# agent-charon/MinGraph-UNet

Measured on AMD Instinct MI355X. Metric: segmented Mpix/sec, full MinGraph-UNet forward (U-Net + patch-graph GAT), 512x512 batch, higher is better.
Workload: dtype f32

## Files before the change

mingraph-unet_amd/csrc/common.h:

```cpp
#pragma once
#include <hip/hip_runtime.h>
#include <stdint.h>

#include "device.h"

namespace mgu {

inline int grid_for(int64_t work, int threads, int cap) {
  int64_t b = (work + threads - 1) / threads;
  if (b < 1) b = 1;
  if (b > cap) b = cap;
  return (int)b;
}
inline bool aligned16(const void* p) { return ((uintptr_t)p & 15) == 0; }

struct Tuning {
  bool first_mfma = true;
  bool use_wino = true;
  int wino_prec = 1;
  bool convt_frag = true;
  bool wino_cp = true;
  int wino_ppb_cap = 32;
  bool wgrad_halo = true;
  bool wino_wgrad = true;
  bool convt_dgrad_x3 = true;
  bool wgrad_x3 = true;
  bool wgrad_thin = true;
  bool wino_dgrad = true;
  bool gat_fused = true;
  bool head_fused = true;
  bool wino_asm = true;
};
const Tuning& default_tuning();
hipError_t ensure_dyn_lds(const void* func, size_t bytes, bool (&done)[64]);

struct IgemmDesc {
  const Tuning* tn;
  const float* in;
  const float* w;
  const float* wu;
  const float* scale;
  const float* shift;
  float* out;
  int M;
  int H, W;
  int Cp;
  int ldin;
  int KS;
  int K;
  int Kp;
  int N;
  int ldout;
  int coff;
  int relu;
  int out_mode;
  int ct_cout;
  int Hout, Wout;
  float* pool;
  int ldpool;
  double* stat_slots;
  int split_n;
  float* out2;
  int ld2;
};

struct WinoHead {
  const float* w;
  const float* b;
  float* logits;
  float* psum;
  int ncls;
  int psum_bytes;
};
inline size_t wino_head_psum_bytes(int B, int H, int W) { return (size_t)B * (H / 16) * (W / 16) * 8 * 32 * sizeof(float); }

inline const Tuning& tun(const IgemmDesc& d) { return d.tn ? *d.tn : default_tuning(); }
enum class ConvKernel {
  None,
  WinoAsmWide, WinoAsmCp1r2, WinoAsmCp1r4,
  WinoAsmCp1r2Head,
  WinoCp2, WinoCp1, WinoCp2Stats, WinoCp1Stats,
  WinoCp1Head,
  WinoF32Wide, WinoF32Narrow,
  WinoX3Wide, WinoX3Narrow,
  HaloF32, HaloBf16Np8, HaloBf16Np4,
  TilesF32, TilesBf16,
  ConvtX3, ConvtBf16f, ConvtX3Dgrad,
};
ConvKernel pick_conv(const IgemmDesc& d, int dtype, const WinoHead* head = nullptr);
hipError_t launch_conv(const IgemmDesc& d, ConvKernel k, int dtype, hipStream_t s, const WinoHead* head = nullptr);
inline bool conv_fuses_head(ConvKernel k) { return k == ConvKernel::WinoAsmCp1r2Head || k == ConvKernel::WinoCp1Head; }
inline hipError_t launch_igemm_f32(const IgemmDesc& d, hipStream_t s) { return launch_conv(d, pick_conv(d, 0), 0, s); }
inline hipError_t launch_igemm_bf16(const IgemmDesc& d, hipStream_t s) { return launch_conv(d, pick_conv(d, 1), 1, s); }
const char* conv_kernel_name(ConvKernel k, const IgemmDesc& d);
const char* conv_dgrad_name(ConvKernel k, const IgemmDesc& d);
struct ConvCost {
  double mfma;
  int pipe;
};
ConvCost conv_cost(ConvKernel k, const IgemmDesc& d);
inline bool conv_is_wino(ConvKernel k) { return k >= ConvKernel::WinoAsmWide && k <= ConvKernel::WinoX3Narrow; }
inline bool conv_fuses_pool(ConvKernel k) {
  return conv_is_wino(k) || (k >= ConvKernel::HaloF32 && k <= ConvKernel::HaloBf16Np4);
}
inline bool conv_reads_panel(ConvKernel k) {
  return !conv_is_wino(k) && k != ConvKernel::ConvtX3 && k != ConvKernel::ConvtBf16f && k != ConvKernel::ConvtX3Dgrad;
}
bool wino_layer(const Tuning& t, int KS, int Cp);
bool wino_dgrad_layer(const Tuning& t, int KS, int Cop);
bool convt_x3_layer(const Tuning& t, int Cin, int Cout);
bool convt_x3_dgrad_layer(const Tuning& t, int Cin, int Cout);
bool convt_bf16f_layer(const Tuning& t, int Cin, int Cout);
bool wino_head_layer(const Tuning& t, int dtype, int Cin, int ncls, int patch, int B, int H, int W);
inline bool wino_wide(const IgemmDesc& d) { return d.N > 32; }
struct WinoPlan {
  int tiles_x, tiles_y, total, nblk, ppb, ngroups, per_xcd;
};
WinoPlan wino_plan(const IgemmDesc& d);
int wino_grid_blocks(const IgemmDesc& d);
hipError_t launch_convt_x3(const IgemmDesc& d, hipStream_t s);
hipError_t launch_convt_bf16f(const IgemmDesc& d, hipStream_t s);
hipError_t launch_convt_x3_dgrad(const IgemmDesc& d, hipStream_t s);
bool first_mfma_applicable(int dtype, int Cin, int Cp, int Cout, int ldout, int coff, int64_t H, int64_t W);
hipError_t launch_first_mfma(int dtype, const void* in, const float* wfm, const float* scale, const float* shift, void* out, int B, int H,
                             int W, int ldout, int coff, int relu, hipStream_t s);
hipError_t launch_first_mfma_direct(int dtype, const float* x, int64_t sn, int64_t sc, int64_t sh, int64_t sw, int cin, const float* wfm,
                                    const float* scale, const float* shift, void* out, int B, int H, int W, int ldout, int coff, int relu,
                                    hipStream_t s);
bool first_conv_applicable(int dtype, int Cin, int Cp, int Cout, int ldout, int coff);
hipError_t launch_first_conv(int dtype, const void* in, const float* wf, const float* scale, const float* shift, void* out, int B, int H, int W,
                             int Cin, int Cout, int ldout, int coff, int relu, hipStream_t s);
hipError_t launch_wino_f32(const IgemmDesc& d, ConvKernel k, hipStream_t s, const WinoHead* head = nullptr);
hipError_t launch_patch_sum_combine(const float* psum, float* out, int nodes, hipStream_t s);
hipError_t launch_wino_cp_asm(const IgemmDesc& d, ConvKernel k, hipStream_t s, const WinoHead* head = nullptr);

struct PackItem {
  const float* w;
  float* U;
  int Cout, Cin, Cp, Np, dgrad;
  unsigned blk0;
  int kind;
  int mode;
};
static_assert(sizeof(PackItem) == 48, "PackItem must have no padding");
PackItem pack_wino(const float* w, float* U, int Cout, int Cin, int Cp, int dgrad, int prec);
PackItem pack_first_w(const float* w, float* wf, int Cout, int Cin);
PackItem pack_first_mfma(const float* w, float* wfm, int Cout, int Cin);
PackItem pack_convt_x3(const float* w, float* Wx, int Cin, int Cout, int dgrad);
PackItem pack_bias_tile(const float* bias, float* shift, int C, int reps);
PackItem pack_dgrad_panel(const float* w, float* wp, int Cout, int Cin, int Cop, int KS, int Kp);
PackItem pack_conv_panel(const float* w, void* wp, int dtype, int Cout, int Cin, int Cp, int KS, int Kp);
PackItem pack_convt_panel(const float* w, void* wp, int dtype, int Cin, int Cout, int Kp);
PackItem pack_convt_bf16f(const float* w, float* Wf, int Cin, int Cout);
PackItem pack_convt_dgrad_panel(const float* w, float* wp, int Cin, int Cout, int Kp);
size_t wino_u_floats(int Cout, int Cp);
size_t convt_x3_floats(int Cin, int Cout);
size_t convt_x3_dgrad_floats(int Cin, int Cout);
size_t convt_bf16f_floats(int Cin, int Cout);
size_t first_mfma_floats();
constexpr int PACK_MAX = 64;
struct PackBatch {
  int n;
  unsigned total_blocks;
  PackItem it[PACK_MAX];
};
bool pack_batch_prepare(PackBatch& b);
hipError_t launch_pack_batch(const PackBatch* batch_dev, unsigned total_blocks, hipStream_t s);
hipError_t launch_pack_one(const PackItem& it, hipStream_t s);

struct WgradDesc {
  const Tuning* tn;
  const float* z;
  int ldz, zoff;
  const float* in;
  int ldin, inoff, Cp;
  int KS;
  int M, H, W;
  int Hs, Ws;
  int N, K, Kp;
  float* dw;
  size_t dw_capacity;
  int groups;
  int rows_per_split;
};
inline const Tuning& tun(const WgradDesc& d) { return d.tn ? *d.tn : default_tuning(); }
enum class WgradKernel {
  Thin,
  WinoX3,
  Wino,
  Halo,
  Tiles,
};
WgradKernel pick_wgrad(const WgradDesc& d);
const char* wgrad_kernel_name(WgradKernel k);
struct WgradCost {
  double mfma;
  int pipe;
};
WgradCost wgrad_cost(WgradKernel k, double alg);
hipError_t launch_wgrad_f32(WgradDesc& d, hipStream_t s);
hipError_t launch_wino_wgrad_f32(WgradDesc& d, bool x3, hipStream_t s);
hipError_t launch_wgrad_thin(WgradDesc& d, hipStream_t s);

constexpr int STAT_ROWS = 576;
constexpr int CHAN_REDUCE_ROWS = 512;
size_t chan_reduce_work_bytes(int Cmax);
hipError_t launch_bn_stats(const float* z, int ldz, int64_t M, int C, double* work, double* sums, hipStream_t s);
hipError_t launch_bn_finalize(const double* sum, const double* sumsq, int64_t M, float eps, float momentum,
                              const float* gamma, const float* beta, float* mean, float* invstd, float* scale,
                              float* shift, float* run_mean, float* run_var, int C, hipStream_t s);
hipError_t launch_bn_finalize_slots(double* slots, int nrows, double* sums, int64_t M, float eps, float momentum, const float* gamma,
                                    const float* beta, float* mean, float* invstd, float* scale, float* shift, float* run_mean,
                                    float* run_var, int C, hipStream_t s);
hipError_t launch_bn_apply_relu(const float* z, const float* scale, const float* shift, float* y, int ldy, int64_t M, int C,
                                hipStream_t s);
hipError_t launch_bn_apply_relu_pool(const float* z, const float* scale, const float* shift, float* y, int ldy, float* pooled, int B, int H,
                                     int W, int C, hipStream_t s);
hipError_t launch_bn_bwd_reduce(const float* dy, int lddy, const float* fwd_scale, const float* fwd_shift, const float* z, int ldz,
                                const float* mean, const float* invstd, int64_t M, int C, double* work, double* sums,
                                float* dbeta, float* dgamma, hipStream_t s);
hipError_t launch_bn_bwd_apply(const float* dy, int lddy, const float* fwd_scale, const float* fwd_shift, const float* z, const float* mean,
                               const float* invstd, const float* gamma, const double* sums, int64_t M, int C, float* dz,
                               double* work, float* dbias, hipStream_t s);
hipError_t launch_bn_bwd_apply_deferred(const float* dy, int lddy, const float* fsc, const float* fsh, const float* z, const float* mean,
                                        const float* invstd, const float* gamma, const double* sums, int64_t M, int C, float* dz,
                                        double* work, int* rows, hipStream_t s);
hipError_t launch_colsum(const float* z, int ldz, int64_t M, int C, double* work, float* out, hipStream_t s);
hipError_t launch_maxpool2_bwd_add(const float* y, int ldy, const float* dpool, float* dskip, int ldd, int B, int H, int W,
                                   int C, hipStream_t s);
hipError_t launch_zero_pad_region(float* buf, int ld, int coff, int C, int B, int H, int W, int h2, int w2, hipStream_t s);
hipError_t launch_ce(const float* logits, const int64_t* labels, int64_t M, int C, long long ignore_index, float grad_scale,
                     float* dlogits, int ldd, double* acc, int* err_word, float* loss_out, hipStream_t s);
hipError_t launch_unpack_conv_grad(const float* dwp, int groups, size_t panel_stride, float* g, int Cout, int Cin, int Cp, int KS,
                                   int Kp, hipStream_t s, double* fold_slots = nullptr, int fold_rows = 0, int fold_n = 0, float* fold_out = nullptr);
hipError_t launch_unpack_convt_grad(const float* dwp, int groups, size_t panel_stride, float* g, int Cin, int Cout, int Kp, hipStream_t s);
hipError_t launch_sgd(float* p, const float* g, float* buf, int64_t n, float lr, float momentum, float wd, int step, float grad_scale,
                      hipStream_t s);
hipError_t launch_adam(float* p, const float* g, float* m, float* v, int64_t n, float lr, float b1, float b2, float eps,
                       float wd, int step, float grad_scale, hipStream_t s);

hipError_t launch_pack_input(const float* x, void* out, int dtype, int B, int C, int Cp, int H, int W, int64_t sn, int64_t sc,
                             int64_t sh, int64_t sw, hipStream_t s);
hipError_t launch_maxpool2(const void* in, int ldin, void* out, int dtype, int B, int H, int W, int C, hipStream_t s);
bool patch_mean_head_fusable(int dtype, int C, int ncls);
hipError_t launch_patch_mean(const void* feat, int dtype, float* out, int B, int H, int W, int C, int patch, hipStream_t s,
                             const float* head_w = nullptr, const float* head_b = nullptr, float* logits = nullptr, int ncls = 0);
hipError_t launch_bn_fold(const float* bias, const float* gamma, const float* beta, const float* mean, const float* var,
                          float eps, float* scale, float* shift, int C, hipStream_t s);
hipError_t launch_conv1x1_head(const void* in, int dtype, int ldin, int C, const float* w, const float* bias, float* out,
                               int ldout, int ncls, int64_t npix, hipStream_t s);
hipError_t launch_argmax(const float* logits, int64_t npix, int C, int64_t* pred, hipStream_t s);

hipError_t launch_gat_wa_rows(const float* W, const float* a, float* panel, int row0, int heads, int Fh, int Fin, int Kp, hipStream_t s);
bool gat_fused_applicable(int Fin, int heads, int Fh, int64_t E);
size_t gat_fused_scratch_floats(int Fin, int heads, int Fh);
hipError_t launch_gat_prep(const float* W, const float* a, float* wa, unsigned* Wx, int heads, int Fh, int Fin, hipStream_t s);
hipError_t launch_gat_stmax(const float* x, const float* wa, int N, int Fin, int heads, const int32_t* rowptr, const int32_t* col,
                            const int32_t* gp, int G, float alpha, float* st, int32_t* node_graph, unsigned long long* gmax, int gstride,
                            unsigned gen, hipStream_t s);
hipError_t launch_gat_fused(const float* x, int Fin, const float* st, const int32_t* rowptr, const int32_t* col, const int32_t* gp, int G,
                            const unsigned long long* gmax, const unsigned* Wx, int N, int heads, int Fh, int concat, float alpha, float* out,
                            int gstride, unsigned gen, hipStream_t s);
hipError_t launch_gat_node_graph(const int32_t* gp, int G, int nodes_per_graph, int N, int32_t* node_graph, hipStream_t s);
hipError_t launch_gat_edge_max(const float* st, const int32_t* rowptr, const int32_t* col, const int32_t* node_graph, int N,
                               int heads, float alpha, unsigned long long* gmax_enc, int gstride, unsigned gen, hipStream_t s);
hipError_t launch_gat_aggregate(const float* wh, int P, const float* st, const int32_t* rowptr, const int32_t* col,
                                const int32_t* node_graph, const unsigned long long* gmax_enc, int N, int64_t E, int heads, int Fh,
                                int concat, float alpha, float* out, int gstride, unsigned gen, hipStream_t s);

}
```

mingraph-unet_amd/csrc/convt_x3.hip:

```cpp
#include <hip/hip_runtime.h>
#include <stdint.h>

#include <algorithm>
#include <type_traits>

#include "common.h"

namespace mgu {


namespace {

template <int MODE, int NI>
__global__ __launch_bounds__(256, 2) void convt2x2_x3_kernel(const float* __restrict__ in, const int ldin, const uint16_t* __restrict__ Wx,
                                                             const float* __restrict__ shift, float* __restrict__ out, const int M,
                                                             const int H, const int W, const int Cin, const int Cout, const int ldout,
                                                             const int coff, const int Hout, const int Wout, const int ntn,
                                                             const int nblocks) {
  constexpr int AP = 40, ABUF = 3 * 128 * AP;
  __shared__ __attribute__((aligned(16))) uint16_t As[2 * ABUF];
  __shared__ int rowoff[128];
  const int chunk = gridDim.x >> 3;
  const int lb = (blockIdx.x & 7) * chunk + (blockIdx.x >> 3);
  if (lb >= nblocks) return;
  const int nt = lb % ntn, mt = lb / ntn;
  const int tid = threadIdx.x, lane = tid & 63, wave = tid >> 6;
  const int wm = wave >> 1, wn = wave & 1, lr = lane & 31, lh = lane >> 5;
  const int bm0 = mt * 128;
  const int HW = H * W;
  long long pix0;
  {
    const int img = bm0 / HW, rem = bm0 - img * HW, y = rem / W;
    pix0 = ((long long)img * Hout + 2 * y) * Wout + 2 * (rem - y * W);
  }
  if (tid < 128) {
    const int m = bm0 + tid;
    int off = 0;
    if (m < M) {
      const int img = m / HW, rem = m - img * HW, y = rem / W, x = rem - y * W;
      off = (int)((((long long)img * Hout + 2 * y) * Wout + 2 * x - pix0) * ldout);
    }
    rowoff[tid] = off;
  }

  const int arow = tid >> 3, ach = (tid & 7) * 4;
  const float* aptr[4];
#pragma unroll
  for (int j = 0; j < 4; ++j) {
    const int m = min(bm0 + j * 32 + arow, M - 1);
    if (MODE == 0) {
      aptr[j] = in + (size_t)m * ldin + ach;
    } else {
      const int img = m / HW, rem = m - img * HW, y = rem / W, x = rem - y * W;
      aptr[j] = in + (((size_t)img * Hout + 2 * y) * Wout + 2 * x) * ldin + ach;
    }
  }
  const int nk = (MODE == 0 ? Cin : 4 * Cin) >> 5;
  const int spq = Cin >> 5;
  auto koff = [&](int s) -> int {
    if (MODE == 0) return s * 32;
    const int q = s / spq;
    return ((q >> 1) * Wout + (q & 1)) * ldin + (s - q * spq) * 32;
  };
  f32x4 areg[2][4];
  auto load_a = [&](int s, auto set_t) {
    constexpr int set = decltype(set_t)::value;
    const int ko = koff(s);
#pragma unroll
    for (int j = 0; j < 4; ++j) areg[set][j] = *reinterpret_cast<const f32x4*>(aptr[j] + ko);
  };
  auto store_a = [&](int buf, auto set_t) {
    constexpr int set = decltype(set_t)::value;
    uint16_t* const base = As + buf * ABUF + arow * AP + ach;
#pragma unroll
    for (int j = 0; j < 4; ++j) {
      unsigned p[3][2];
      split3_pack(areg[set][j][0], areg[set][j][1], p[0][0], p[1][0], p[2][0]);
      split3_pack(areg[set][j][2], areg[set][j][3], p[0][1], p[1][1], p[2][1]);
#pragma unroll
      for (int q = 0; q < 3; ++q) *reinterpret_cast<uint2*>(base + (q * 128 + j * 32) * AP) = uint2{p[q][0], p[q][1]};
    }
  };

  const int nt128 = NI == 2 ? nt : nt >> 1, sub0 = NI == 2 ? wn * 2 : (nt & 1) * 2 + wn;
  const u32x4* const bp = reinterpret_cast<const u32x4*>(Wx) + ((size_t)nt128 * (2 * nk) * 12 + sub0 * 3) * 64 + lane;
  u32x4 br[2][3 * NI];
  auto load_b = [&](int kk, auto buf_t) {
    constexpr int buf = decltype(buf_t)::value;
#pragma unroll
    for (int f = 0; f < 3 * NI; ++f) br[buf][f] = bp[((size_t)kk * 12 + f) * 64];
  };

  f32x16 acc[2][NI];
#pragma unroll
  for (int mi = 0; mi < 2; ++mi)
#pragma unroll
    for (int ni = 0; ni < NI; ++ni)
#pragma unroll
      for (int r = 0; r < 16; ++r) acc[mi][ni][r] = 0.f;

  const int aoff = (wm * 64 + lr) * AP + lh * 8;
  auto half_step = [&](int buf, int ss, auto bb_t) {
    constexpr int bb = decltype(bb_t)::value;
    u32x4 pa[2][3];
#pragma unroll
    for (int mi = 0; mi < 2; ++mi)
#pragma unroll
      for (int q = 0; q < 3; ++q)
        pa[mi][q] = *reinterpret_cast<const u32x4*>(As + buf * ABUF + (q * 128 + mi * 32) * AP + aoff + ss * 16);
#pragma unroll
    for (int mi = 0; mi < 2; ++mi)
#pragma unroll
      for (int ni = 0; ni < NI; ++ni) {
        f32x16 t = acc[mi][ni];
        t = mfma_bf16(pa[mi][2], br[bb][ni * 3 + 0], t);
        t = mfma_bf16(pa[mi][0], br[bb][ni * 3 + 2], t);
        t = mfma_bf16(pa[mi][1], br[bb][ni * 3 + 1], t);
        t = mfma_bf16(pa[mi][1], br[bb][ni * 3 + 0], t);
        t = mfma_bf16(pa[mi][0], br[bb][ni * 3 + 1], t);
        t = mfma_bf16(pa[mi][0], br[bb][ni * 3 + 0], t);
        acc[mi][ni] = t;
      }
  };
  using B0 = std::integral_constant<int, 0>;
  using B1 = std::integral_constant<int, 1>;
  const int nkk = 2 * nk;
  load_a(0, B0{});
  load_a(min(1, nk - 1), B1{});
  load_b(0, B0{});
  store_a(0, B0{});
  lds_barrier();
  auto second_half_and_stage = [&](int buf, auto bb_t, auto set_t) {
    half_step(buf, 1, bb_t);
    store_a(buf ^ 1, set_t);
#pragma unroll
    for (int k = 0; k < 12 * NI; ++k) {
      __builtin_amdgcn_sched_group_barrier(0x008, 1, 0);
      __builtin_amdgcn_sched_group_barrier(0x002, NI == 2 ? 4 : 8, 0);
    }
    __builtin_amdgcn_sched_group_barrier(0x200, 12, 0);
  };
  for (int s = 0; s < nk; s += 2) {
    load_a(min(s + 2, nk - 1), B0{});
    load_b(min(2 * s + 1, nkk - 1), B1{});
    __builtin_amdgcn_sched_barrier(0);
    half_step(0, 0, B0{});
    load_b(min(2 * s + 2, nkk - 1), B0{});
    __builtin_amdgcn_sched_barrier(0);
    second_half_and_stage(0, B1{}, B1{});
    __builtin_amdgcn_sched_barrier(0);
    lds_barrier();
    if (s + 1 >= nk) break;
    load_a(min(s + 3, nk - 1), B1{});
    load_b(min(2 * s + 3, nkk - 1), B1{});
    __builtin_amdgcn_sched_barrier(0);
    half_step(1, 0, B0{});
    load_b(min(2 * s + 4, nkk - 1), B0{});
    __builtin_amdgcn_sched_barrier(0);
    second_half_and_stage(1, B1{}, B0{});
    __builtin_amdgcn_sched_barrier(0);
    lds_barrier();
  }

  float* const tile_out = MODE == 0 ? out + (size_t)pix0 * ldout + coff : out + (size_t)bm0 * ldout + coff;
  const bool full_m = bm0 + 128 <= M;
  auto store_tile = [&](auto guarded_t) {
    constexpr bool GUARDED = decltype(guarded_t)::value;
#pragma unroll
    for (int ni = 0; ni < NI; ++ni) {
      const int n = nt * (64 * NI) + wn * (32 * NI) + ni * 32 + lr;
      int ncol = n;
      if (MODE == 0) {
        const int q = n / Cout;
        ncol = ((q >> 1) * Wout + (q & 1)) * ldout + (n - q * Cout);
      }
      const float sh = shift ? shift[n] : 0.f;
#pragma unroll
      for (int mi = 0; mi < 2; ++mi)
#pragma unroll
        for (int r = 0; r < 16; ++r) {
          const int rrow = wm * 64 + mi * 32 + (r & 3) + 8 * (r >> 2) + 4 * lh;
          const unsigned idx = (unsigned)((MODE == 0 ? rowoff[rrow] : rrow * ldout) + ncol);
          const float v = acc[mi][ni][r] + sh;
          if (!GUARDED) tile_out[idx] = v;
          else if (bm0 + rrow < M) tile_out[idx] = v;
        }
    }
  };
  if (full_m) store_tile(std::false_type{});
  else store_tile(std::true_type{});
}

}

hipError_t launch_convt_x3_dgrad(const IgemmDesc& d, hipStream_t s) {
  const bool wide = (d.N & 127) == 0;
  const int mtiles = (d.M + 127) / 128, ntn = d.N / (wide ? 128 : 64);
  const int nb = mtiles * ntn;
  const int chunk = (nb + 7) / 8;
  if (wide)
    hipLaunchKernelGGL((convt2x2_x3_kernel<1, 2>), dim3(chunk * 8), dim3(256), 0, s, d.in, d.ldin, reinterpret_cast<const uint16_t*>(d.wu),
                       (const float*)nullptr, d.out, d.M, d.H, d.W, d.Cp, d.N, d.ldout, d.coff, d.Hout, d.Wout, ntn, nb);
  else
    hipLaunchKernelGGL((convt2x2_x3_kernel<1, 1>), dim3(chunk * 8), dim3(256), 0, s, d.in, d.ldin, reinterpret_cast<const uint16_t*>(d.wu),
                       (const float*)nullptr, d.out, d.M, d.H, d.W, d.Cp, d.N, d.ldout, d.coff, d.Hout, d.Wout, ntn, nb);
  return hipGetLastError();
}

hipError_t launch_convt_x3(const IgemmDesc& d, hipStream_t s) {
  const int mtiles = (d.M + 127) / 128, ntn = d.N / 128;
  const int nb = mtiles * ntn;
  const int chunk = (nb + 7) / 8;
  hipLaunchKernelGGL((convt2x2_x3_kernel<0, 2>), dim3(chunk * 8), dim3(256), 0, s, d.in, d.ldin, reinterpret_cast<const uint16_t*>(d.wu), d.shift, d.out,
                     d.M, d.H, d.W, d.Cp, d.ct_cout, d.ldout, d.coff, d.Hout, d.Wout, ntn, nb);
  return hipGetLastError();
}

}
```

mingraph-unet_amd/csrc/device.h:

```cpp
#pragma once
#include <hip/hip_runtime.h>
#include <stdint.h>
#include <type_traits>

namespace mgu {

typedef float f32x16 __attribute__((ext_vector_type(16)));
typedef float f32x4 __attribute__((ext_vector_type(4)));
typedef float f32x2 __attribute__((ext_vector_type(2)));
typedef unsigned u32x4 __attribute__((ext_vector_type(4)));
typedef unsigned u32x2 __attribute__((ext_vector_type(2)));
typedef __bf16 bf16x8 __attribute__((ext_vector_type(8)));

__device__ __forceinline__ void split3_pack(const float a, const float b, unsigned& p0, unsigned& p1, unsigned& p2) {
  const unsigned ua = __float_as_uint(a), ub = __float_as_uint(b);
  p0 = __builtin_amdgcn_perm(ub, ua, 0x07060302u);
  const float ra = a - __uint_as_float(ua & 0xffff0000u), rb = b - __uint_as_float(ub & 0xffff0000u);
  const unsigned va = __float_as_uint(ra), vb = __float_as_uint(rb);
  p1 = __builtin_amdgcn_perm(vb, va, 0x07060302u);
  const float sa = ra - __uint_as_float(va & 0xffff0000u), sb = rb - __uint_as_float(vb & 0xffff0000u);
  p2 = __builtin_amdgcn_perm(__float_as_uint(sb), __float_as_uint(sa), 0x07060302u);
}
__device__ __forceinline__ float x3_add(float a, float b) {
  float d;
  asm("v_add_f32 %0, %1, %2" : "=v"(d) : "v"(a), "v"(b));
  return d;
}
__device__ __forceinline__ float x3_sub(float a, float b) {
  float d;
  asm("v_sub_f32 %0, %1, %2" : "=v"(d) : "v"(a), "v"(b));
  return d;
}
__device__ __forceinline__ float x3_fma(float a, float b, float c) {
  float d;
  asm("v_fma_f32 %0, %1, %2, %3" : "=v"(d) : "v"(a), "v"(b), "v"(c));
  return d;
}
__device__ __forceinline__ void split3_pack_s(const float a, const float b, unsigned& p0, unsigned& p1, unsigned& p2) {
  const unsigned ua = __float_as_uint(a), ub = __float_as_uint(b);
  p0 = __builtin_amdgcn_perm(ub, ua, 0x07060302u);
  const float ra = x3_sub(a, __uint_as_float(ua & 0xffff0000u)), rb = x3_sub(b, __uint_as_float(ub & 0xffff0000u));
  const unsigned va = __float_as_uint(ra), vb = __float_as_uint(rb);
  p1 = __builtin_amdgcn_perm(vb, va, 0x07060302u);
  const float sa = x3_sub(ra, __uint_as_float(va & 0xffff0000u)), sb = x3_sub(rb, __uint_as_float(vb & 0xffff0000u));
  p2 = __builtin_amdgcn_perm(__float_as_uint(sb), __float_as_uint(sa), 0x07060302u);
}

__device__ __forceinline__ f32x16 mfma_bf16(const u32x4 a, const u32x4 b, const f32x16 c) {
  return __builtin_amdgcn_mfma_f32_32x32x16_bf16(__builtin_bit_cast(bf16x8, a), __builtin_bit_cast(bf16x8, b), c, 0, 0, 0);
}

template <int I, int N, class F>
__device__ __forceinline__ void static_for(F&& f) {
  if constexpr (I < N) {
    f(std::integral_constant<int, I>{});
    static_for<I + 1, N>(f);
  }
}

__device__ __forceinline__ void lds_barrier() { asm volatile("s_waitcnt lgkmcnt(0)\n\ts_barrier" ::: "memory"); }
__device__ __forceinline__ void lds_barrier_builtin() {
  asm volatile("" ::: "memory");
  __builtin_amdgcn_s_waitcnt(0xC07F);
  __builtin_amdgcn_s_barrier();
  asm volatile("" ::: "memory");
}
__device__ __forceinline__ void lds_barrier_fenced() { __syncthreads(); }

template <typename T>
__device__ __forceinline__ T wave_sum(T v) {
#pragma unroll
  for (int off = 32; off > 0; off >>= 1) v += __shfl_xor(v, off);
  return v;
}
__device__ __forceinline__ int wave_min(int v) {
#pragma unroll
  for (int off = 32; off > 0; off >>= 1) v = min(v, __shfl_xor(v, off));
  return v;
}
__device__ __forceinline__ int wave_max(int v) {
#pragma unroll
  for (int off = 32; off > 0; off >>= 1) v = max(v, __shfl_xor(v, off));
  return v;
}
template <int K>
__device__ __forceinline__ void block_fold(double (&v)[K], double* sh ) {
#pragma unroll
  for (int k = 0; k < K; ++k)
#pragma unroll
    for (int off = 32; off > 0; off >>= 1) v[k] += __shfl_xor(v[k], off);
  const int lane = threadIdx.x & 63, wave = threadIdx.x >> 6;
  if (lane == 0)
#pragma unroll
    for (int k = 0; k < K; ++k) sh[wave * K + k] = v[k];
  __syncthreads();
  if (threadIdx.x == 0)
#pragma unroll
    for (int k = 0; k < K; ++k) v[k] = sh[k] + sh[K + k] + sh[2 * K + k] + sh[3 * K + k];
}

__device__ __forceinline__ unsigned enc_ordered(float f) {
  const unsigned u = __float_as_uint(f);
  return (u & 0x80000000u) ? ~u : (u | 0x80000000u);
}
__device__ __forceinline__ float dec_ordered(unsigned u) {
  return __uint_as_float((u & 0x80000000u) ? (u & 0x7FFFFFFFu) : ~u);
}

template <int CM>
__device__ __forceinline__ float pixel_softmax(const float* p, int C, float (&e)[CM]) {
  float l[CM];
  float m = p[0];
#pragma unroll
  for (int c = 0; c < CM; ++c)
    if (c < C) {
      l[c] = p[c];
      m = fmaxf(m, l[c]);
    }
  float sum = 0.f;
#pragma unroll
  for (int c = 0; c < CM; ++c)
    if (c < C) {
      e[c] = expf(l[c] - m);
      sum += e[c];
    }
  return sum;
}
__device__ __forceinline__ float u8_normalize(uint8_t u, int c, float m0, float m1, float m2, float s0, float s1, float s2) {
  const float v = (float)u / 255.f;
  const float mean = c == 0 ? m0 : (c == 1 ? m1 : m2), sd = c == 0 ? s0 : (c == 1 ? s1 : s2);
  return (v - mean) / sd;
}

__device__ __forceinline__ int graph_of(const int32_t* __restrict__ gp, int G, int node) {
  if (!gp || G <= 1) return 0;
  int lo = 0, hi = G;
  while (hi - lo > 1) {
    const int mid = (lo + hi) >> 1;
    if (gp[mid] <= node) lo = mid; else hi = mid;
  }
  return lo;
}

}
```

mingraph-unet_amd/csrc/igemm.hip:

```cpp
#include "common.h"
#include <algorithm>
#include <type_traits>

namespace mgu {


const Tuning& default_tuning() {
  static const Tuning t;
  return t;
}

hipError_t ensure_dyn_lds(const void* func, size_t bytes, bool (&done)[64]) {
  if (bytes <= 65536) return hipSuccess;
  int dev = 0;
  hipError_t e = hipGetDevice(&dev);
  if (e != hipSuccess) return e;
  if (dev < 0 || dev >= 64) return hipFuncSetAttribute(func, hipFuncAttributeMaxDynamicSharedMemorySize, (int)bytes);
  if (done[dev]) return hipSuccess;
  e = hipFuncSetAttribute(func, hipFuncAttributeMaxDynamicSharedMemorySize, (int)bytes);
  if (e == hipSuccess) done[dev] = true;
  return e;
}

template <typename T> struct Elem;
template <> struct Elem<float> { static constexpr int VEC = 4; };
template <> struct Elem<__bf16> { static constexpr int VEC = 8; };

template <typename T>
__device__ __forceinline__ f32x16 mma_chunk(const f32x4 a, const f32x4 b, f32x16 c) {
  if constexpr (sizeof(T) == 4) {
#pragma unroll
    for (int t = 0; t < 4; ++t) c = __builtin_amdgcn_mfma_f32_32x32x2f32(a[t], b[t], c, 0, 0, 0);
    return c;
  } else {
    return __builtin_amdgcn_mfma_f32_32x32x16_bf16(__builtin_bit_cast(bf16x8, a), __builtin_bit_cast(bf16x8, b), c, 0, 0, 0);
  }
}

template <typename T, int KS, int OUTMODE, int WAVES_M, int WAVES_N, int WMT, int WNT>
__global__ __launch_bounds__(256) void igemm_kernel(const IgemmDesc d) {
  static_assert(WAVES_M * WAVES_N == 4, "4 wavefronts per workgroup");
  constexpr int VEC = Elem<T>::VEC;
  constexpr int CK = 8 * VEC;
  constexpr int LDS_LD = CK + VEC;
  constexpr int BM = WAVES_M * WMT * 32;
  constexpr int BN = WAVES_N * WNT * 32;
  constexpr int AR = BM / 32;
  constexpr int BR = BN / 32;
  extern __shared__ __attribute__((aligned(16))) float smem_raw[];
  T* smem = reinterpret_cast<T*>(smem_raw);
  T* As = smem;
  T* Bs = smem + BM * LDS_LD;
  const T* const in_t = reinterpret_cast<const T*>(d.in);
  const T* const w_t = reinterpret_cast<const T*>(d.w);

  const int tid = threadIdx.x;
  const int lane = tid & 63;
  const int wave = tid >> 6;
  const int wm = wave / WAVES_N;
  const int wn = wave % WAVES_N;
  const int bm0 = blockIdx.x * BM;
  const int bn0 = blockIdx.y * BN;
  const int kq = tid & 7;
  const int r0 = tid >> 3;

  const T* abase[AR];
  unsigned amask[AR];
  const int HW = d.H * d.W;
#pragma unroll
  for (int i = 0; i < AR; ++i) {
    const int m = bm0 + r0 + 32 * i;
    abase[i] = in_t;
    amask[i] = 0u;
    if (m < d.M) {
      abase[i] = in_t + (size_t)m * d.ldin;
      if (KS == 2) {
        const int img = m / HW;
        const int rem = m - img * HW;
        const int oy = rem / d.W;
        const int ox = rem - oy * d.W;
        abase[i] = in_t + (((size_t)img * d.Hout + 2 * oy) * d.Wout + 2 * ox) * d.ldin;
        amask[i] = 0xFu;
      } else if (KS == 3) {
        const int rem = m % HW;
        const int oy = rem / d.W;
        const int ox = rem - oy * d.W;
        unsigned rowok = (oy > 0 ? 1u : 0u) | 2u | (oy + 1 < d.H ? 4u : 0u);
        unsigned colok = (ox > 0 ? 1u : 0u) | 2u | (ox + 1 < d.W ? 4u : 0u);
        unsigned mk = 0u;
#pragma unroll
        for (int r = 0; r < 3; ++r)
          if (rowok & (1u << r)) mk |= colok << (3 * r);
        amask[i] = mk;
      } else {
        amask[i] = 1u;
      }
    }
  }
  const T* wrow[BR];
#pragma unroll
  for (int i = 0; i < BR; ++i) wrow[i] = w_t + (size_t)(bn0 + r0 + 32 * i) * d.Kp + kq * VEC;

  f32x4 areg[AR];
  f32x4 breg[BR];
  auto load_tiles = [&](int k0) {
    const int k = k0 + kq * VEC;
    int tap = 0;
    long delta = k;
    if (KS == 3) {
      tap = k / d.Cp;
      const int c = k - tap * d.Cp;
      const int r = tap / 3;
      const int s = tap - 3 * r;
      delta = (long)((r - 1) * d.W + (s - 1)) * d.ldin + c;
    } else if (KS == 2) {
      tap = k / d.Cp;
      const int c = k - tap * d.Cp;
      delta = (long)((tap >> 1) * d.Wout + (tap & 1)) * d.ldin + c;
    }
    const bool kvalid = k < d.K;
#pragma unroll
    for (int i = 0; i < AR; ++i) {
      const bool ok = kvalid && ((amask[i] >> tap) & 1u);
      const T* src = ok ? abase[i] + delta : in_t;
      const f32x4 v = *reinterpret_cast<const f32x4*>(src);
      areg[i] = ok ? v : f32x4{0.f, 0.f, 0.f, 0.f};
    }
#pragma unroll
    for (int i = 0; i < BR; ++i) breg[i] = *reinterpret_cast<const f32x4*>(wrow[i] + k0);
  };

  f32x16 acc[WMT][WNT];
#pragma unroll
  for (int mi = 0; mi < WMT; ++mi)
#pragma unroll
    for (int ni = 0; ni < WNT; ++ni)
#pragma unroll
      for (int r = 0; r < 16; ++r) acc[mi][ni][r] = 0.f;

  const int lr = lane & 31;
  const int lh = lane >> 5;
  const T* Ap = As + (wm * WMT * 32 + lr) * LDS_LD + lh * VEC;
  const T* Bp = Bs + (wn * WNT * 32 + lr) * LDS_LD + lh * VEC;
  T* Asw = As + r0 * LDS_LD + kq * VEC;
  T* Bsw = Bs + r0 * LDS_LD + kq * VEC;

  const int nk = d.Kp / CK;
  load_tiles(0);
  for (int ks = 0; ks < nk; ++ks) {
#pragma unroll
    for (int i = 0; i < AR; ++i) *reinterpret_cast<f32x4*>(Asw + i * 32 * LDS_LD) = areg[i];
#pragma unroll
    for (int i = 0; i < BR; ++i) *reinterpret_cast<f32x4*>(Bsw + i * 32 * LDS_LD) = breg[i];
    __syncthreads();
    if (ks + 1 < nk) load_tiles((ks + 1) * CK);
#pragma unroll
    for (int kk = 0; kk < 4; ++kk) {
      if (ks * CK + kk * 2 * VEC >= d.K) break;
      f32x4 a[WMT], b[WNT];
#pragma unroll
      for (int mi = 0; mi < WMT; ++mi) a[mi] = *reinterpret_cast<const f32x4*>(Ap + mi * 32 * LDS_LD + kk * 2 * VEC);
#pragma unroll
      for (int ni = 0; ni < WNT; ++ni) b[ni] = *reinterpret_cast<const f32x4*>(Bp + ni * 32 * LDS_LD + kk * 2 * VEC);
#pragma unroll
      for (int mi = 0; mi < WMT; ++mi)
#pragma unroll
        for (int ni = 0; ni < WNT; ++ni) acc[mi][ni] = mma_chunk<T>(a[mi], b[ni], acc[mi][ni]);
    }
    __syncthreads();
  }

  int* rowoff = reinterpret_cast<int*>(smem_raw);
  long long pix0 = 0;
  if (OUTMODE == 1) {
    {
      const int img = bm0 / HW;
      const int rem = bm0 - img * HW;
      const int y = rem / d.W;
      pix0 = ((long long)img * d.Hout + 2 * y) * d.Wout + 2 * (rem - y * d.W);
    }
    for (int rrow = tid; rrow < BM; rrow += 256) {
      const int m = bm0 + rrow;
      int off = 0;
      if (m < d.M) {
        const int img = m / HW;
        const int rem = m - img * HW;
        const int y = rem / d.W;
        const int x = rem - y * d.W;
        off = (int)((((long long)img * d.Hout + 2 * y) * d.Wout + 2 * x - pix0) * d.ldout);
      }
      rowoff[rrow] = off;
    }
    __syncthreads();
  }
  const bool full_m = bm0 + BM <= d.M;
  const bool full_n = bn0 + BN <= d.N;
  T* const out_t = reinterpret_cast<T*>(d.out);
  T* const tile_out = OUTMODE == 1 ? out_t + (size_t)pix0 * d.ldout + d.coff : out_t + (size_t)bm0 * d.ldout + d.coff;
  auto store_tile = [&](auto guarded_t) {
    constexpr bool GUARDED = decltype(guarded_t)::value;
#pragma unroll
    for (int ni = 0; ni < WNT; ++ni) {
      const int n = bn0 + (wn * WNT + ni) * 32 + lr;
      const bool nvalid = n < d.N;
      const float sc = (nvalid && d.scale) ? d.scale[n] : 1.f;
      const float sh = (nvalid && d.shift) ? d.shift[n] : 0.f;
      int ncol = n;
      if (OUTMODE == 1) {
        const int q = n / d.ct_cout;
        ncol = ((q >> 1) * d.Wout + (q & 1)) * d.ldout + (n - q * d.ct_cout);
      }
      const bool split = OUTMODE == 0 && d.split_n > 0 && n >= d.split_n;
#pragma unroll
      for (int mi = 0; mi < WMT; ++mi) {
#pragma unroll
        for (int r = 0; r < 16; ++r) {
          const int row = (r & 3) + 8 * (r >> 2) + 4 * lh;
          const int rrow = (wm * WMT + mi) * 32 + row;
          float v = acc[mi][ni][r] * sc + sh;
          if (d.relu) v = fmaxf(v, 0.f);
          const unsigned idx = OUTMODE == 1 ? (unsigned)(rowoff[rrow] + ncol) : (unsigned)(rrow * d.ldout + ncol);
          if (!GUARDED) {
            tile_out[idx] = (T)v;
          } else if (nvalid && (full_m || bm0 + rrow < d.M)) {
            if (split) d.out2[(size_t)(bm0 + rrow) * d.ld2 + (n - d.split_n)] = v;
            else tile_out[idx] = (T)v;
          }
        }
      }
    }
  };
  if (full_m && full_n && !(OUTMODE == 0 && d.split_n > 0)) store_tile(std::false_type{});
  else store_tile(std::true_type{});
}

__device__ __forceinline__ float max_1op(const float lo, const float x) {
  float r;
  asm("v_max_f32_e32 %0, %1, %2" : "=v"(r) : "v"(lo), "v"(x));
  return r;
}

template <int N>
__device__ __forceinline__ void wait_vmcnt() {
  __builtin_amdgcn_s_waitcnt((N & 15) | ((N >> 4) << 14) | 0x70 | 0xF00);
}

template <typename T, int NP, int TH, int WAVES_M, int WAVES_N, int WMT, int WNT, int TPS>
__global__ __launch_bounds__(256, 2) void conv3x3_halo_kernel(const IgemmDesc d, const int tiles_x, const int tiles_y,
                                                           const int total_patches, const int patches_per_block) {
  constexpr int VEC = Elem<T>::VEC;
  constexpr int CK = NP * VEC;
  constexpr int LDS_LD = CK + VEC;
  constexpr int RPP = 256 / NP;
  static_assert(TPS == 1 || TPS == 3, "taps per step");
  constexpr int SPI = 9 / TPS;
  constexpr int TW = 16, HWID = TW + 2, HP = (TH + 2) * HWID;
  constexpr int BM = TH * TW;
  constexpr int BN = WAVES_N * WNT * 32;
  static_assert(BM == WAVES_M * WMT * 32 && WAVES_M * WAVES_N == 4, "tile/wave mismatch");
  constexpr int HR = (HP + RPP - 1) / RPP;
  constexpr int BR = (BN + RPP - 1) / RPP;
  extern __shared__ __attribute__((aligned(16))) float smem_raw[];
  T* Hs = reinterpret_cast<T*>(smem_raw);
  T* Bs = Hs + HP * LDS_LD;
  constexpr bool GLDS = NP == 8 && BN % 32 == 0;
  constexpr int BROW = GLDS ? CK : LDS_LD;
  constexpr int NBUF = (GLDS && (HP * LDS_LD + 3 * TPS * BN * CK) * (int)sizeof(T) <= 80 * 1024) ? 3 : 2;
  constexpr int NGL = TPS * (BN / 32);
  const T* const in_t = reinterpret_cast<const T*>(d.in);
  const T* const w_t = reinterpret_cast<const T*>(d.w);

  const int tid = threadIdx.x;
  const int lane = tid & 63;
  const int wave = tid >> 6;
  const int wm = wave / WAVES_N;
  const int wn = wave % WAVES_N;
  const int kq = tid % NP;
  const int r0 = tid / NP;
  const int bn0 = blockIdx.y * BN;
  const int p_begin = blockIdx.x * patches_per_block;
  const int npatch = min(patches_per_block, total_patches - p_begin);
  if (npatch <= 0) return;

  int hoff[HR];
  auto in_rsrc = __builtin_amdgcn_make_buffer_rsrc(const_cast<T*>(in_t), 0, 0x7ffffff0, 0x00020000);
  const unsigned img_bytes = (unsigned)((size_t)d.H * d.W * d.ldin * sizeof(T));
  struct PatchPos { int img, y0, x0; };
  auto setup_patch = [&](int p) {
    const int ty = (p / tiles_x) % tiles_y;
    const int tx = p % tiles_x;
    return PatchPos{p / (tiles_x * tiles_y), ty * TH, tx * TW};
  };
  auto setup_load = [&](int p) {
    const PatchPos pp = setup_patch(p);
    const int img = pp.img, y0 = pp.y0, x0 = pp.x0;
    in_rsrc = __builtin_amdgcn_make_buffer_rsrc(const_cast<T*>(in_t) + (size_t)img * d.H * d.W * d.ldin, 0, img_bytes, 0x00020000);
#pragma unroll
    for (int i = 0; i < HR; ++i) {
      const int hp = r0 + RPP * i;
      const int hy = hp / HWID, hx = hp - hy * HWID;
      const int y = y0 - 1 + hy, x = x0 - 1 + hx;
      const bool ok = hp < HP && y >= 0 && y < d.H && x >= 0 && x < d.W;
      hoff[i] = ok ? ((y * d.W + x) * d.ldin + kq * VEC) * (int)sizeof(T) : 0x7fff0000;
    }
  };
  const T* wrow[BR];
#pragma unroll
  for (int i = 0; i < BR; ++i) wrow[i] = w_t + (size_t)(bn0 + r0 + RPP * i) * d.Kp + kq * VEC;

  constexpr bool DEEPH = NP == 4 && HR <= 6;
  constexpr int NSETH = DEEPH ? 2 : 1;
  f32x4 hreg[NSETH][HR];
  f32x4 breg[TPS][BR];
  auto load_halo = [&](int c, auto set_c) {
    constexpr int set = decltype(set_c)::value;
#pragma unroll
    for (int i = 0; i < HR; ++i)
      hreg[set][i] = __builtin_bit_cast(f32x4, __builtin_amdgcn_raw_buffer_load_b128(in_rsrc, hoff[i], c * CK * (int)sizeof(T), 0));
  };
  auto store_halo = [&](auto set_c) {
    constexpr int set = decltype(set_c)::value;
#pragma unroll
    for (int i = 0; i < HR; ++i)
      if (r0 + RPP * i < HP) *reinterpret_cast<f32x4*>(Hs + (r0 + RPP * i) * LDS_LD + kq * VEC) = hreg[set][i];
  };
  auto load_b = [&](int c, int stp) {
#pragma unroll
    for (int tt = 0; tt < TPS; ++tt) {
      const int k0 = (stp * TPS + tt) * d.Cp + c * CK;
#pragma unroll
      for (int i = 0; i < BR; ++i) breg[tt][i] = *reinterpret_cast<const f32x4*>(wrow[i] + k0);
    }
  };
  auto glds_b = [&](int c, int stp, int buf) {
    if constexpr (GLDS) {
      const int wave_u = __builtin_amdgcn_readfirstlane(wave);
#pragma unroll
      for (int tt = 0; tt < TPS; ++tt) {
        const int k0 = (stp * TPS + tt) * d.Cp + c * CK;
#pragma unroll
        for (int j = 0; j < BN / 32; ++j) {
          const int ii = wave_u * (BN / 32) + j;
          const int row = 8 * ii + (lane >> 3);
          const int logical = (lane & 7) ^ ((row >> 1) & 7);
          const T* src = w_t + (size_t)(bn0 + row) * d.Kp + k0 + logical * VEC;
          T* dst = Bs + ((size_t)(buf * TPS + tt) * BN + 8 * ii) * BROW;
#if defined(__HIP_DEVICE_COMPILE__)
          __builtin_amdgcn_global_load_lds(src, dst, 16, 0, 0);
#else
          (void)src, (void)dst;
#endif
        }
      }
    }
  };
  auto store_b = [&](int buf) {
#pragma unroll
    for (int tt = 0; tt < TPS; ++tt)
#pragma unroll
      for (int i = 0; i < BR; ++i)
        if (BN % RPP == 0 || r0 + RPP * i < BN)
          *reinterpret_cast<f32x4*>(Bs + ((buf * TPS + tt) * BN + r0 + RPP * i) * LDS_LD + kq * VEC) = breg[tt][i];
  };

  f32x16 acc[WMT][WNT];
#pragma unroll
  for (int mi = 0; mi < WMT; ++mi)
#pragma unroll
    for (int ni = 0; ni < WNT; ++ni)
#pragma unroll
      for (int r = 0; r < 16; ++r) acc[mi][ni][r] = 0.f;

  const int lr = lane & 31;
  const int lh = lane >> 5;
  int aoff[WMT];
#pragma unroll
  for (int mi = 0; mi < WMT; ++mi) {
    const int pp = (wm * WMT + mi) * 32 + lr;
    aoff[mi] = ((pp >> 4) * HWID + (pp & 15)) * LDS_LD + lh * VEC;
  }
  const int boff = GLDS ? (wn * WNT * 32 + lr) * BROW : (wn * WNT * 32 + lr) * LDS_LD + lh * VEC;
  const int bswz = ((wn * WNT * 32 + lr) >> 1) & 7;

  const int nchunks = d.Cp / CK;
  const int nitems = npatch * nchunks;
  using Set0 = std::integral_constant<int, 0>;
  using Set1 = std::integral_constant<int, DEEPH ? 1 : 0>;
  int li = 0;
  auto load_next_halo = [&](auto set_c) {
    const int lic = min(li, nitems - 1);
    const int lp = lic / nchunks, lc = lic - lp * nchunks;
    if (lc == 0 && li < nitems) setup_load(p_begin + lp);
    load_halo(lc, set_c);
    ++li;
  };
  auto wg_barrier = [&]() {
    if constexpr (GLDS) {
      lds_barrier_builtin();
    } else {
      __syncthreads();
    }
  };
  constexpr int STORES_PER_INTERIOR_PATCH = WMT * WNT * 16;
  constexpr int NST = STORES_PER_INTERIOR_PATCH < 63 ? STORES_PER_INTERIOR_PATCH : 63;
  static_assert(NST <= STORES_PER_INTERIOR_PATCH && NST <= 63, "vmcnt count above the stores really issued");
  int w0 = 0;
  load_next_halo(Set0{});
  if constexpr (GLDS) {
    glds_b(0, 0, 0);
    if constexpr (NBUF == 3) glds_b(0, 1, 1);
    store_halo(Set0{});
    wait_vmcnt<0>();
  } else {
    load_b(0, 0);
    store_halo(Set0{});
    store_b(0);
    load_b(0, 1);
  }
  if constexpr (DEEPH) load_next_halo(Set1{});
  int c = 0, pi = 0;
  int par = 0;
  auto do_item = [&](auto par_c) {
    using SetLoad = std::integral_constant<int, DEEPH ? decltype(par_c)::value : 0>;
    using SetStore = std::integral_constant<int, DEEPH ? (decltype(par_c)::value ^ 1) : 0>;
    const int cnext = c + 1 == nchunks ? 0 : c + 1;
    static_for<0, SPI>([&](auto tap_c) {
      constexpr int tap = decltype(tap_c)::value;
      if constexpr (GLDS) {
        constexpr int HRL = HR < 63 ? HR : 63;
        if constexpr (NBUF == 2) {
          if constexpr (tap == 1) wait_vmcnt<HRL>();
          else if constexpr (tap == 0) {
            if (w0) wait_vmcnt<NST>();
            else wait_vmcnt<0>();
          } else wait_vmcnt<0>();
        } else {
          constexpr int both = NGL + HRL < 63 ? NGL + HRL : 63;
          if constexpr (tap == 1 || tap == 2) wait_vmcnt<both>();
          else wait_vmcnt<NGL>();
        }
      }
      wg_barrier();
      if constexpr (GLDS) {
        constexpr int ahead = NBUF - 1;
        const int tgt = NBUF == 2 ? (par ^ 1) : (par == 0 ? 2 : par - 1);
        if constexpr (tap + ahead < SPI) glds_b(c, tap + ahead, tgt);
        else glds_b(cnext, tap + ahead - SPI, tgt);
        if constexpr (tap == 0) load_next_halo(SetLoad{});
      }
    {
      constexpr int NKK = NP / 2;
      constexpr int NG = TPS * NKK;
      constexpr int DEPTH = (GLDS && NG == 4 && HR <= 6) ? 4 : (NG >= 3 && HR * NSETH <= 12) ? 3 : 2;
      f32x4 a[DEPTH][WMT], b[DEPTH][WNT];
      auto fetch = [&](int gidx, int slot) {
        const int tt = gidx / NKK, kk = gidx % NKK;
        const int tp = tap * TPS + tt;
        const int r = tp / 3, s = tp - 3 * r;
        const T* Ap = Hs + (r * HWID + s) * LDS_LD + kk * 2 * VEC;
        const T* Bp = GLDS ? Bs + (par * TPS + tt) * BN * BROW + boff + (((2 * kk + lh) ^ bswz) * VEC)
                           : Bs + (par * TPS + tt) * BN * LDS_LD + boff + kk * 2 * VEC;
#pragma unroll
        for (int mi = 0; mi < WMT; ++mi) a[slot][mi] = *reinterpret_cast<const f32x4*>(Ap + aoff[mi]);
#pragma unroll
        for (int ni = 0; ni < WNT; ++ni) b[slot][ni] = *reinterpret_cast<const f32x4*>(Bp + ni * 32 * BROW);
      };
#pragma unroll
      for (int gidx = 0; gidx < DEPTH - 1; ++gidx) fetch(gidx, gidx);
      __builtin_amdgcn_sched_barrier(0);
#pragma unroll
      for (int gidx = 0; gidx < NG; ++gidx) {
        if (gidx + DEPTH - 1 < NG) {
          fetch(gidx + DEPTH - 1, (gidx + DEPTH - 1) % DEPTH);
          __builtin_amdgcn_sched_barrier(0);
        }
#pragma unroll
        for (int mi = 0; mi < WMT; ++mi)
#pragma unroll
          for (int ni = 0; ni < WNT; ++ni) acc[mi][ni] = mma_chunk<T>(a[gidx % DEPTH][mi], b[gidx % DEPTH][ni], acc[mi][ni]);
      }
    }
      if constexpr (!GLDS) {
        store_b(par ^ 1);
        if constexpr (tap + 2 < SPI) load_b(c, tap + 2);
        else load_b(cnext, tap + 2 - SPI);
        if constexpr (tap == 0) load_next_halo(SetLoad{});
      }
      if constexpr (NBUF == 2) par ^= 1;
      else par = par == 2 ? 0 : par + 1;
    });
    {
      const bool patch_done = (c + 1 == nchunks);
      const bool more = patch_done ? (pi + 1 < npatch) : true;
      if (more) {
        wg_barrier();
        store_halo(SetStore{});
      }
      w0 = 0;
      if (patch_done) {
        const PatchPos pp = setup_patch(p_begin + pi);
        const int img = pp.img, y0 = pp.y0, x0 = pp.x0;
        T* const img_out = reinterpret_cast<T*>(d.out) + (size_t)img * d.H * d.W * d.ldout + d.coff;
        const bool interior = (y0 + TH <= d.H) && (x0 + TW <= d.W) && (bn0 + BN <= d.N);
        const unsigned sA = (unsigned)(d.W * d.ldout), sB = (unsigned)d.ldout;
        const auto out_rsrc = __builtin_amdgcn_make_buffer_rsrc(img_out, 0, 0x7ffffff0, 0x00020000);
        const int wm_s = __builtin_amdgcn_readfirstlane(wm);
        const float relu_lo = d.relu ? 0.f : __builtin_nanf("");
        auto store_patch = [&](auto guarded_t) {
          constexpr bool GUARDED = decltype(guarded_t)::value;
#pragma unroll
          for (int ni = 0; ni < WNT; ++ni) {
            const int n = bn0 + (wn * WNT + ni) * 32 + lr;
            const bool nvalid = n < d.N;
            const float sc = (nvalid && d.scale) ? d.scale[n] : 1.f;
            const float sh = (nvalid && d.shift) ? d.shift[n] : 0.f;
            const unsigned lane_idx = (unsigned)((y0 * d.W + x0 + 4 * lh) * d.ldout + n);
#pragma unroll
            for (int mi = 0; mi < WMT; ++mi) {
              float vv[16];
#pragma unroll
              for (int rr = 0; rr < 16; ++rr) {
                const int pyc = 2 * (wm * WMT + mi) + (rr >> 3);
                const int pxc = 8 * ((rr >> 2) & 1) + (rr & 3);
                float v = acc[mi][ni][rr] * sc + sh;
                v = max_1op(relu_lo, v);
                vv[rr] = v;
                const unsigned idx = lane_idx + (unsigned)pyc * sA + (unsigned)pxc * sB;
                if (!GUARDED) {
                  const int soff = (int)(((unsigned)(2 * (wm_s * WMT + mi) + (rr >> 3)) * sA + (unsigned)pxc * sB) * (unsigned)sizeof(T));
                  if constexpr (sizeof(T) == 2)
                    __builtin_amdgcn_raw_buffer_store_b16(__builtin_bit_cast(unsigned short, (T)v), out_rsrc, (int)(lane_idx * 2u), soff, 0);
                  else
                    __builtin_amdgcn_raw_buffer_store_b32(__builtin_bit_cast(unsigned, v), out_rsrc, (int)(lane_idx * 4u), soff, 0);
                } else if (nvalid && y0 + pyc < d.H && x0 + pxc + 4 * lh < d.W) {
                  img_out[idx] = (T)v;
                }
                acc[mi][ni][rr] = 0.f;
              }
              if (d.pool) {
                T* const pool_img = reinterpret_cast<T*>(d.pool) + (size_t)img * (d.H >> 1) * (d.W >> 1) * d.ldpool;
#pragma unroll
                for (int a = 0; a < 8; a += 2) {
                  const float m = max_1op(max_1op(vv[a], vv[a + 1]), max_1op(vv[a + 8], vv[a + 9]));
                  const int pyc = 2 * (wm * WMT + mi), pxc = 8 * ((a >> 2) & 1) + (a & 3) + 4 * lh;
                  const int py = (y0 + pyc) >> 1, px = (x0 + pxc) >> 1;
                  if (!GUARDED || (nvalid && y0 + pyc + 1 < d.H && x0 + pxc + 1 < d.W))
                    pool_img[((size_t)py * (d.W >> 1) + px) * d.ldpool + n] = (T)m;
                }
              }
            }
          }
        };
        if (interior) store_patch(std::false_type{});
        else store_patch(std::true_type{});
        w0 = interior ? 1 : 0;
      }
      pi += patch_done ? 1 : 0;
      c = patch_done ? 0 : c + 1;
    }
  };
  for (int item = 0; item < nitems; item += NSETH) {
    do_item(Set0{});
    if constexpr (DEEPH) {
      if (item + 1 < nitems) do_item(Set1{});
    }
  }
}

template <typename T, int NP, int TH, int WAVES_M, int WAVES_N, int WMT, int WNT, int TPS>
static hipError_t launch_halo(const IgemmDesc& d, hipStream_t s) {
  constexpr int BN = WAVES_N * WNT * 32;
  constexpr int HP = (TH + 2) * 18;
  const int tiles_x = (d.W + 15) / 16, tiles_y = (d.H + TH - 1) / TH;
  const int B = d.M / (d.H * d.W);
  const int total = tiles_x * tiles_y * B, ntn = (d.N + BN - 1) / BN;
  const int ppb = std::min(std::max((int)(((long)total * ntn) / (256 * 4)), 1), 16);
  dim3 grid((total + ppb - 1) / ppb, ntn);
  size_t lds = (size_t)(HP + 2 * TPS * BN) * (NP * 16 + 16);
  if (NP == 8 && BN % 32 == 0 && (size_t)HP * (NP * 16 + 16) + (size_t)3 * TPS * BN * NP * 16 <= 80 * 1024)
    lds = (size_t)HP * (NP * 16 + 16) + (size_t)3 * TPS * BN * NP * 16;
  static bool attr_done[64] = {};
  hipError_t ae = ensure_dyn_lds(reinterpret_cast<const void*>(&conv3x3_halo_kernel<T, NP, TH, WAVES_M, WAVES_N, WMT, WNT, TPS>), lds, attr_done);
  if (ae != hipSuccess) return ae;
  hipLaunchKernelGGL((conv3x3_halo_kernel<T, NP, TH, WAVES_M, WAVES_N, WMT, WNT, TPS>), grid, dim3(256), lds, s, d, tiles_x,
                     tiles_y, total, ppb);
  return hipGetLastError();
}

template <typename T>
static int halo_np(const IgemmDesc& d) {
  constexpr int VEC = Elem<T>::VEC;
  if (!(d.KS == 3 && d.out_mode == 0 && d.K == 9 * d.Cp && d.ldin == d.Cp && (long)d.H * d.W * d.ldin * (long)sizeof(T) < 0x7fff0000l &&
        (long)d.H * d.W * d.ldout * (long)sizeof(T) < 0x7ffffff0l))
    return 0;
  if (d.Cp % (8 * VEC) == 0) return 8;
  if (sizeof(T) == 2 && d.Cp % (4 * VEC) == 0) return 4;
  return 0;
}

template <typename T, int KS, int OUTMODE, int WAVES_M, int WAVES_N, int WMT, int WNT>
static hipError_t launch_cfg(const IgemmDesc& d, hipStream_t s) {
  constexpr int BM = WAVES_M * WMT * 32;
  constexpr int BN = WAVES_N * WNT * 32;
  dim3 grid((d.M + BM - 1) / BM, (d.N + BN - 1) / BN);
  const size_t lds = (size_t)(BM + BN) * 144;
  hipLaunchKernelGGL((igemm_kernel<T, KS, OUTMODE, WAVES_M, WAVES_N, WMT, WNT>), grid, dim3(256), lds, s, d);
  return hipGetLastError();
}

template <typename T, int KS, int OUTMODE>
static hipError_t launch_tiles(const IgemmDesc& d, hipStream_t s) {
  if (d.N > 64) return launch_cfg<T, KS, OUTMODE, 2, 2, 2, 2>(d, s);
  if (d.N > 32) return launch_cfg<T, KS, OUTMODE, 4, 1, 2, 2>(d, s);
  return launch_cfg<T, KS, OUTMODE, 4, 1, 2, 1>(d, s);
}

template <typename T, int NP>
static hipError_t launch_halo_tiles(const IgemmDesc& d, hipStream_t s) {
  if (d.N > 64) return launch_halo<T, NP, 8, 2, 2, 2, 2, 1>(d, s);
  if (d.N > 32) return launch_halo<T, NP, 16, 4, 1, 2, 2, 1>(d, s);
  return launch_halo<T, NP, 16, 4, 1, 2, 1, 3>(d, s);
}

bool wino_layer(const Tuning& t, int KS, int Cp) { return t.use_wino && KS == 3 && Cp % 16 == 0; }
bool wino_dgrad_layer(const Tuning& t, int KS, int Cop) { return t.wino_dgrad && wino_layer(t, KS, Cop); }
bool convt_x3_layer(const Tuning& t, int Cin, int Cout) { return t.wino_prec != 0 && t.convt_frag && Cin % 32 == 0 && Cout % 32 == 0; }
bool convt_x3_dgrad_layer(const Tuning& t, int Cin, int Cout) {
  return t.wino_prec != 0 && t.convt_dgrad_x3 && Cin % 64 == 0 && Cout % 32 == 0;
}
bool convt_bf16f_layer(const Tuning& t, int Cin, int Cout) { return t.convt_frag && Cin % 64 == 0 && Cout % 32 == 0; }

static bool wino_applicable(const IgemmDesc& d) {
  return wino_layer(tun(d), d.KS, d.Cp) && d.wu && d.out_mode == 0 && d.split_n == 0 && d.K == 9 * d.Cp && (d.ldin & 3) == 0 &&
         (long)d.H * d.W * d.ldin < (1l << 31) && (long)d.H * d.W * d.ldout < (1l << 31);
}

static bool wino_asm_shape(const IgemmDesc& d) {
  if (d.stat_slots) return false;
  if (wino_wide(d)) {
    if (d.N & 63) return false;
  } else {
    if (d.N != 32 || !(d.Cp == 32 || d.Cp == 64)) return false;
  }
  if ((d.H & 7) || (d.W & 31) || (d.Cp & 31) || (d.ldin & 3) || (d.ldout & 3) || (d.coff & 3)) return false;
  if (d.pool && ((d.ldpool & 3) || (d.H & 1) || (d.W & 1))) return false;
  if ((long)d.H * d.W * d.ldin * 4 >= 0x7fff0000l || (long)d.H * d.W * d.ldout * 4 >= 0x7fff0000l) return false;
  const WinoPlan p = wino_plan(d);
  if ((long)p.total * p.tiles_x * p.tiles_y >= (1l << 32) || (long)p.ngroups * p.nblk * p.ngroups >= (1l << 32)) return false;
  return true;
}

static bool wino_asm_applicable(const IgemmDesc& d) { return tun(d).wino_asm && wino_asm_shape(d); }

bool wino_head_layer(const Tuning& t, int dtype, int Cin, int ncls, int patch, int B, int H, int W) {
  if (!t.head_fused || dtype != 0 || Cin != 32 || ncls < 1 || ncls > 4 || patch != 16 || B < 1 || (H & 15) || (W & 31)) return false;
  return (long)H * W * ncls * 4 < 0x7fff0000l && wino_head_psum_bytes(B, H, W) < 0x7fff0000ul;
}

static bool wino_head_applicable(const IgemmDesc& d, const WinoHead& h) {
  const int B = (int)(d.M / ((long)d.H * d.W));
  if (!wino_head_layer(tun(d), 0, d.Cp, h.ncls, 16, B, d.H, d.W)) return false;
  if (!wino_asm_shape(d) || wino_wide(d) || d.pool || d.ldout != 32 || d.coff) return false;
  return h.w && h.b && h.logits && h.psum && (size_t)h.psum_bytes == wino_head_psum_bytes(B, d.H, d.W);
}

static bool convt_x3_applicable(const IgemmDesc& d) {
  return convt_x3_layer(tun(d), d.Cp, d.ct_cout) && d.wu && d.KS == 1 && d.K == d.Cp && d.N == 4 * d.ct_cout && (d.ldin & 3) == 0 &&
         !d.scale && !d.relu && !d.split_n && (9l * 128 + 8l * d.Wout) * d.ldout < (1l << 31);
}

static bool convt_bf16f_applicable(const IgemmDesc& d) {
  return convt_bf16f_layer(tun(d), d.Cp, d.ct_cout) && d.wu && d.KS == 1 && d.K == d.Cp && d.N == 4 * d.ct_cout && (d.ldin & 7) == 0 &&
         (d.ldout & 7) == 0 && (d.coff & 7) == 0 && !d.scale && !d.relu && !d.split_n &&
         (9l * 128 + 8l * d.Wout) * d.ldout < (1l << 31);
}

static bool convt_x3_dgrad_applicable(const IgemmDesc& d) {
  return convt_x3_dgrad_layer(tun(d), d.N, d.Cp) && d.KS == 2 && d.wu && d.K == 4 * d.Cp && (d.ldin & 3) == 0 && !d.scale && !d.shift &&
         !d.relu && !d.split_n && !d.pool && (long)d.M * d.ldout < (1l << 31) && (long)d.Hout * d.Wout * d.ldin < (1l << 31);
}

ConvKernel pick_conv(const IgemmDesc& d, int dtype, const WinoHead* head) {
  using K = ConvKernel;
  if (d.M <= 0 || d.N <= 0) return K::None;
  if (dtype == 1) {
    if (d.out_mode == 1) return d.KS != 1 ? K::None : convt_bf16f_applicable(d) ? K::ConvtBf16f : K::TilesBf16;
    const int np = halo_np<__bf16>(d);
    if (np) return np == 8 ? K::HaloBf16Np8 : K::HaloBf16Np4;
    return d.KS == 3 || d.KS == 1 ? K::TilesBf16 : K::None;
  }
  if (d.out_mode == 1) return d.KS != 1 ? K::None : convt_x3_applicable(d) ? K::ConvtX3 : K::TilesF32;
  if (convt_x3_dgrad_applicable(d)) return K::ConvtX3Dgrad;
  if (wino_applicable(d)) {
    const Tuning& t = tun(d);
    const bool wide = wino_wide(d);
    if (!t.wino_prec) return wide ? K::WinoF32Wide : K::WinoF32Narrow;
    if (!t.wino_cp || (long)d.H * d.W * d.ldin * 4 >= 0x7fff0000l) return wide ? K::WinoX3Wide : K::WinoX3Narrow;
    if (d.stat_slots) return wide ? K::WinoCp2Stats : K::WinoCp1Stats;
    if (head && wino_head_applicable(d, *head)) return t.wino_asm ? K::WinoAsmCp1r2Head : K::WinoCp1Head;
    if (wino_asm_applicable(d)) return wide ? K::WinoAsmWide : d.Cp == 32 ? K::WinoAsmCp1r2 : K::WinoAsmCp1r4;
    return wide ? K::WinoCp2 : K::WinoCp1;
  }
  if (halo_np<float>(d) == 8) return K::HaloF32;
  return d.KS >= 1 && d.KS <= 3 ? K::TilesF32 : K::None;
}

const char* conv_kernel_name(ConvKernel k, const IgemmDesc& d) {
  switch (k) {
    case ConvKernel::WinoAsmWide: return "mgu_wino_cp2_gfx950 (asm form of wino3x3_cp_kernel<2>)";
    case ConvKernel::WinoAsmCp1r2: return "mgu_wino_cp1r2_gfx950 (asm form of wino3x3_cp_kernel<1>)";
    case ConvKernel::WinoAsmCp1r4: return "mgu_wino_cp1r4_gfx950 (asm form of wino3x3_cp_kernel<1>)";
    case ConvKernel::WinoAsmCp1r2Head: return "mgu_wino_cp1r2h_gfx950 (asm form of wino3x3_cp_kernel<1, head>: + 1x1 head + patch sums)";
    case ConvKernel::WinoCp1Head: return "wino3x3_cp_kernel<1, head> (+ 1x1 head + patch sums)";
    case ConvKernel::WinoCp2: case ConvKernel::WinoCp2Stats: return "wino3x3_cp_kernel<2>";
    case ConvKernel::WinoCp1: case ConvKernel::WinoCp1Stats: return "wino3x3_cp_kernel<1>";
    case ConvKernel::WinoF32Wide: return "wino3x3_f32_kernel<0,0>";
    case ConvKernel::WinoF32Narrow: return "wino3x3_f32_kernel<1,0>";
    case ConvKernel::WinoX3Wide: return "wino3x3_f32_kernel<0,1>";
    case ConvKernel::WinoX3Narrow: return "wino3x3_f32_kernel<1,1>";
    case ConvKernel::HaloF32: return "conv3x3_halo_kernel<f32>";
    case ConvKernel::HaloBf16Np8: case ConvKernel::HaloBf16Np4: return "conv3x3_halo_kernel<bf16>";
    case ConvKernel::TilesBf16: return d.out_mode == 1 ? "igemm_kernel<bf16> (ConvTranspose)" : "igemm_kernel<bf16>";
    case ConvKernel::ConvtX3: return "convt2x2_x3_kernel";
    case ConvKernel::ConvtBf16f: return "convt2x2_bf16_kernel";
    case ConvKernel::ConvtX3Dgrad: return "convt2x2_x3_kernel<dgrad>";
    case ConvKernel::TilesF32: case ConvKernel::None: break;
  }
  return d.out_mode == 1 ? "igemm_kernel<f32> (ConvTranspose)" : d.KS == 2 ? "igemm_kernel<f32> (ConvTranspose dgrad)" : "igemm_kernel<f32>";
}

const char* conv_dgrad_name(ConvKernel k, const IgemmDesc& d) {
  switch (k) {
    case ConvKernel::WinoAsmWide: case ConvKernel::WinoCp2: case ConvKernel::WinoCp2Stats: return "wino3x3_cp_kernel<2> (dgrad)";
    case ConvKernel::WinoAsmCp1r2: case ConvKernel::WinoAsmCp1r4: case ConvKernel::WinoCp1: case ConvKernel::WinoCp1Stats:
    case ConvKernel::WinoAsmCp1r2Head: case ConvKernel::WinoCp1Head:
      return "wino3x3_cp_kernel<1> (dgrad)";
    case ConvKernel::WinoX3Wide: case ConvKernel::WinoX3Narrow: return "wino3x3_f32_kernel<*,1> (dgrad)";
    case ConvKernel::WinoF32Wide: case ConvKernel::WinoF32Narrow: return "wino3x3_f32_kernel<*,0> (dgrad)";
    case ConvKernel::ConvtX3Dgrad: return "convt2x2_x3_kernel (dgrad)";
    default: return d.KS == 2 ? "igemm_kernel<f32> (ConvTranspose dgrad)" : "igemm/halo (dgrad)";
  }
}

ConvCost conv_cost(ConvKernel k, const IgemmDesc& d) {
  const double direct = 2.0 * d.M * (double)d.K * d.N;
  switch (k) {
    case ConvKernel::WinoF32Wide: case ConvKernel::WinoF32Narrow:
      return {2.0 * (d.M / (d.H * d.W)) * ((d.H + 1) / 2) * ((d.W + 1) / 2) * 16.0 * d.Cp * d.N, 0};
    case ConvKernel::ConvtX3: case ConvKernel::ConvtX3Dgrad: return {6.0 * direct, 1};
    case ConvKernel::HaloBf16Np8: case ConvKernel::HaloBf16Np4: case ConvKernel::TilesBf16: case ConvKernel::ConvtBf16f: return {direct, 1};
    case ConvKernel::HaloF32: case ConvKernel::TilesF32: case ConvKernel::None: return {direct, 0};
    default:
      return {2.0 * (d.M / (d.H * d.W)) * ((d.H + 1) / 2) * ((d.W + 1) / 2) * 16.0 * d.Cp * d.N * 6.0, 1};
  }
}

hipError_t launch_conv(const IgemmDesc& d, ConvKernel k, int dtype, hipStream_t s, const WinoHead* head) {
  if (d.M <= 0 || d.N <= 0) return hipSuccess;
  if (dtype == 1) {
    if ((d.Cp & 7) || (d.ldin & 7) || (d.Kp % 64) || d.K > d.Kp || d.split_n) return hipErrorInvalidValue;
  } else {
    if ((d.Cp & 3) || (d.ldin & 3) || (d.Kp % 32) || d.K > d.Kp) return hipErrorInvalidValue;
  }
  if (conv_fuses_head(k) != (head != nullptr)) return hipErrorInvalidValue;
  switch (k) {
    case ConvKernel::WinoAsmWide: case ConvKernel::WinoAsmCp1r2: case ConvKernel::WinoAsmCp1r4: return launch_wino_cp_asm(d, k, s);
    case ConvKernel::WinoAsmCp1r2Head: return launch_wino_cp_asm(d, k, s, head);
    case ConvKernel::WinoCp1Head: return launch_wino_f32(d, k, s, head);
    case ConvKernel::WinoCp2: case ConvKernel::WinoCp1: case ConvKernel::WinoCp2Stats: case ConvKernel::WinoCp1Stats:
    case ConvKernel::WinoF32Wide: case ConvKernel::WinoF32Narrow: case ConvKernel::WinoX3Wide: case ConvKernel::WinoX3Narrow:
      return launch_wino_f32(d, k, s);
    case ConvKernel::HaloF32: return launch_halo_tiles<float, 8>(d, s);
    case ConvKernel::HaloBf16Np8: return launch_halo_tiles<__bf16, 8>(d, s);
    case ConvKernel::HaloBf16Np4: return launch_halo_tiles<__bf16, 4>(d, s);
    case ConvKernel::TilesF32:
      if (d.out_mode == 1) return launch_tiles<float, 1, 1>(d, s);
      if (d.KS == 3) return launch_tiles<float, 3, 0>(d, s);
      if (d.KS == 1) return launch_tiles<float, 1, 0>(d, s);
      return launch_tiles<float, 2, 0>(d, s);
    case ConvKernel::TilesBf16:
      if (d.out_mode == 1) return launch_tiles<__bf16, 1, 1>(d, s);
      if (d.KS == 3) return launch_tiles<__bf16, 3, 0>(d, s);
      return launch_tiles<__bf16, 1, 0>(d, s);
    case ConvKernel::ConvtX3: return launch_convt_x3(d, s);
    case ConvKernel::ConvtBf16f: return launch_convt_bf16f(d, s);
    case ConvKernel::ConvtX3Dgrad: return launch_convt_x3_dgrad(d, s);
    case ConvKernel::None: break;
  }
  return hipErrorInvalidValue;
}

}
```

mingraph-unet_amd/csrc/mgunet_api.hip:

```cpp
#include "ctx.h"

#include <algorithm>

using namespace mgu;
using namespace mgud;

namespace mgud {
std::string g_create_err;
}

namespace {

struct WsPlan {
  size_t xin, tmp, bott, total;
  std::vector<size_t> pooled;
};

WsPlan plan_ws(const mgu_ctx* c, int B, int H, int W) {
  std::vector<int> hs, wsz;
  level_dims(H, W, c->depth, hs, wsz);
  auto out = [&](const Block& b, int l) { return (size_t)B * hs[l] * wsz[l] * c->layers[b.conv2].Cout; };
  WsPlan p;
  Carve k;
  const size_t es = c->dtype == MGU_DTYPE_BF16 ? 2 : 4;
  p.xin = k.take((size_t)B * H * W * c->Cp0 * es);
  size_t tmax = out(c->bott, c->bott.level);
  for (const Block& b : c->enc) tmax = std::max(tmax, out(b, b.level));
  p.tmp = k.take(tmax * es);
  for (const Block& b : c->enc) p.pooled.push_back(k.take(out(b, b.level + 1) * es));
  p.bott = k.take(out(c->bott, c->bott.level) * es);
  p.total = k.off;
  return p;
}

template <class F>
void weight_forms(const mgu_ctx* c, Layer& L, F form) {
  const int dtype = c->dtype;
  L.wino = dtype == MGU_DTYPE_F32 && !L.convt && wino_layer(c->tn, L.KS, L.Cp);
  L.ctx3 = dtype == MGU_DTYPE_F32 && L.convt && convt_x3_layer(c->tn, L.Cin, L.Cout);
  L.ctb = dtype == MGU_DTYPE_BF16 && L.convt && convt_bf16f_layer(c->tn, L.Cin, L.Cout);
  L.first = !L.convt && L.KS == 3 && first_conv_applicable(dtype, L.Cin, L.Cp, L.Cout, 8, 0);
  form(L.wp, (size_t)L.Np * L.Kp);
  form(L.scale, (size_t)L.Np);
  form(L.shift, (size_t)L.Np);
  if (L.wino) form(L.wu, wino_u_floats(L.Cout, L.Cp));
  if (L.wino && rup(L.Cout, 4) % 16 == 0) form(L.wug, wino_u_floats(L.Cin, rup(L.Cout, 4)));
  if (L.ctx3) form(L.wu, convt_x3_floats(L.Cin, L.Cout));
  if (L.ctb) form(L.wu, convt_bf16f_floats(L.Cin, L.Cout));
  if (L.ctx3) form(L.wxg, convt_x3_dgrad_floats(L.Cin, L.Cout));
  if (dtype == MGU_DTYPE_F32 && !L.convt && L.bn.empty())
    form(L.wxg, (size_t)rup(L.Cin, 128) * rup(L.KS * L.KS * rup(L.Cout, 4), 32));
  if (L.first) form(L.wf, 9 * 4 * (size_t)L.Cout);
  if (L.first) form(L.wfm, first_mfma_floats());
  if (!L.bn.empty()) {
    form(L.mean, (size_t)L.Np);
    form(L.invstd, (size_t)L.Np);
    form(L.tscale, (size_t)L.Np);
    form(L.tshift, (size_t)L.Np);
  }
}

}

extern "C" {

const char* mgu_version(void) { return "mgunet 0.2 (gfx950: fp32 Winograd / bf16 MFMA forward, fp32 training step, GAT, RCCL gradient exchange)"; }

int mgu_create(int device_id, mgu_ctx** out) {
  if (!out) return fail(nullptr, MGU_ERR_INVALID, "out == NULL");
  int n = 0;
  hipError_t e = hipGetDeviceCount(&n);
  if (e != hipSuccess || n <= 0)
    return fail(nullptr, MGU_ERR_HIP, "no HIP device available (%s): libmgunet has no CPU fallback",
                e != hipSuccess ? hipGetErrorString(e) : "device count 0");
  if (device_id < 0 || device_id >= n) return fail(nullptr, MGU_ERR_INVALID, "device %d out of range [0,%d)", device_id, n);
  e = hipSetDevice(device_id);
  if (e != hipSuccess) return fail(nullptr, MGU_ERR_HIP, "hipSetDevice: %s", hipGetErrorString(e));
  mgu_ctx* c = new mgu_ctx();
  c->device = device_id;
  auto flag = [](const char* name) { const char* v = getenv(name); return v && v[0] == '1'; };
  auto num = [](const char* name, int dflt) { const char* v = getenv(name); return v && v[0] ? atoi(v) : dflt; };
  Tuning& t = c->tn;
  t.first_mfma = !flag("MGU_NO_FIRST_MFMA");
  t.use_wino = !flag("MGU_NO_WINOGRAD");
  t.wino_prec = num("MGU_WINO_PREC", t.wino_prec) ? 1 : 0;
  t.wino_cp = !flag("MGU_NO_WINO_CP");
  t.convt_frag = !flag("MGU_NO_CONVT_FRAG");
  t.wino_ppb_cap = std::max(1, num("MGU_WINO_PPB_CAP", 32));
  t.wgrad_halo = !flag("MGU_NO_WGRAD_HALO");
  t.wino_wgrad = !flag("MGU_NO_WINO_WGRAD");
  t.wgrad_x3 = !flag("MGU_NO_WGRAD_X3");
  t.convt_dgrad_x3 = !flag("MGU_NO_CONVT_DGRAD_X3");
  t.wgrad_thin = !flag("MGU_NO_THIN_WGRAD");
  t.wino_dgrad = !flag("MGU_NO_WINO_DGRAD");
  t.gat_fused = !flag("MGU_NO_GAT_FUSED");
  t.wino_asm = num("MGU_WINO_ASM", 1) > 0;
  t.head_fused = num("MGU_HEAD_FUSED", 1) > 0;
  *out = c;
  return MGU_OK;
}

void mgu_destroy(mgu_ctx* c) {
  if (!c) return;
  (void)hipSetDevice(c->device);
  (void)hipDeviceSynchronize();
  (void)mgu_comm_destroy(c);
  if (c->arena) (void)hipFree(c->arena);
  if (c->ws) (void)hipFree(c->ws);
  if (c->gws) (void)hipFree(c->gws);
  if (c->pmws) (void)hipFree(c->pmws);
  if (c->gbws) (void)hipFree(c->gbws);
  if (c->pack_dev) (void)hipFree(c->pack_dev);
  if (c->tws) (void)hipFree(c->tws);
  if (c->redws) (void)hipFree(c->redws);
  if (c->wuws) (void)hipFree(c->wuws);
  if (c->ncws) (void)hipFree(c->ncws);
  if (c->objws) (void)hipFree(c->objws);
  if (c->lossws) (void)hipFree(c->lossws);
  if (c->imgws) (void)hipFree(c->imgws);
  gat_destroy(c);
  if (c->err_word) (void)hipHostFree(c->err_word);
  for (auto e : c->ev) (void)hipEventDestroy(e);
  for (auto e : c->ev_total)
    if (e) (void)hipEventDestroy(e);
  delete c;
}

const char* mgu_last_error(mgu_ctx* c) { return c ? c->err.c_str() : g_create_err.c_str(); }

int mgu_unet_configure(mgu_ctx* c, int in_ch, int ncls, int feat, int depth, int dtype) {
  if (!c) return MGU_ERR_INVALID;
  if (in_ch < 1 || ncls < 1 || feat < 4 || (feat & 3) || depth < 1 || depth > 8)
    return fail(c, MGU_ERR_INVALID, "unsupported UNet(%d,%d,%d,%d): init_features must be a positive multiple of 4, depth 1..8",
                in_ch, ncls, feat, depth);
  if (dtype != MGU_DTYPE_F32 && dtype != MGU_DTYPE_BF16) return fail(c, MGU_ERR_INVALID, "unknown dtype %d", dtype);
  if (dtype == MGU_DTYPE_BF16 && ((feat & 7) || ncls > 4))
    return fail(c, MGU_ERR_INVALID, "bf16 storage needs init_features %% 8 == 0 (16-byte lanes of 8 bf16) and <= 4 classes");
  HIPCHK(c, hipSetDevice(c->device));
  c->in_ch = in_ch, c->ncls = ncls, c->feat = feat, c->depth = depth, c->dtype = dtype;
  c->Cp0 = rup(in_ch, dtype == MGU_DTYPE_BF16 ? 8 : 4);
  c->layers.clear();
  c->enc.clear();
  c->dec.clear();
  auto add = [&](const std::string& prefix, const char* conv, const char* bn, int cin, int cp, int cout, int KS, bool convt, int level) {
    Layer L;
    L.prefix = prefix, L.conv = conv, L.bn = bn;
    L.Cin = cin, L.Cp = cp, L.Cout = cout, L.KS = KS, L.convt = convt, L.level = level;
    c->layers.push_back(L);
    return (int)c->layers.size() - 1;
  };
  auto add_block = [&](const std::string& prefix, int cin, int cp, int cout, int level, int up) {
    Block b;
    b.up = up, b.level = level;
    b.conv1 = add(prefix, "conv1", "bn1", cin, cp, cout, 3, false, level);
    b.conv2 = add(prefix, "conv2", "bn2", cout, cout, cout, 3, false, level);
    return b;
  };
  int cin = in_ch, cp = c->Cp0, f = feat;
  for (int i = 0; i < depth; ++i) {
    c->enc.push_back(add_block("encoder.encoder_blocks." + std::to_string(i) + ".", cin, cp, f, i, -1));
    cin = cp = f;
    f *= 2;
  }
  c->bott = add_block("encoder.bottleneck.", cin, cp, f, depth, -1);
  int prev = f;
  for (int b = 0; b < depth; ++b) {
    const int i = depth - 1 - b, ci = feat << i;
    const std::string prefix = "decoder.decoder_blocks." + std::to_string(b) + ".";
    const int up = add(prefix, "upsample", "", prev, prev, prev / 2, 1, true, i + 1);
    c->dec.push_back(add_block(prefix + "conv_block.", ci + prev / 2, ci + prev / 2, ci, i, up));
    prev = ci;
  }
  c->head = add("decoder.", "final_conv", "", prev, prev, ncls, 1, false, 0);
  for (auto& L : c->layers) {
    L.K = L.KS * L.KS * L.Cp;
    L.Kp = rup(L.K, dtype == MGU_DTYPE_BF16 ? 64 : 32);
    L.N = L.convt ? 4 * L.Cout : L.Cout;
    L.Np = rup(L.N, 128);
  }
  {
    int64_t off = 0;
    auto conv = [&](Layer& L) {
      L.off_w = off, off += (int64_t)L.Cout * L.Cin * L.KS * L.KS * (L.convt ? 4 : 1);
      L.off_b = off, off += L.Cout;
    };
    auto bn = [&](Layer& L) {
      L.off_gamma = off, off += L.Cout;
      L.off_beta = off, off += L.Cout;
    };
    auto block = [&](const Block& b) {
      if (b.up >= 0) conv(c->layers[b.up]);
      conv(c->layers[b.conv1]), conv(c->layers[b.conv2]);
      bn(c->layers[b.conv1]), bn(c->layers[b.conv2]);
    };
    for (const Block& b : c->enc) block(b);
    block(c->bott);
    for (const Block& b : c->dec) block(b);
    conv(c->layers[c->head]);
    c->nparams = off;
  }
  size_t total = 0;
  for (auto& L : c->layers) weight_forms(c, L, [&](float*&, size_t n) { total += n; });
  if (c->arena) HIPCHK(c, hipFree(c->arena));
  c->arena = nullptr;
  HIPCHK(c, hipMalloc((void**)&c->arena, total * sizeof(float)));
  HIPCHK(c, hipMemset(c->arena, 0, total * sizeof(float)));
  c->arena_floats = total;
  float* p = c->arena;
  for (auto& L : c->layers) weight_forms(c, L, [&](float*& form, size_t n) { form = p, p += n; });
  c->configured = true;
  c->have_train_fwd = false;
  c->loaded = false;
  return MGU_OK;
}

int64_t mgu_unet_param_count(mgu_ctx* c) {
  if (!c || !c->configured) return -1;
  return c->nparams;
}

int64_t mgu_unet_param_offset(mgu_ctx* c, const char* name) {
  if (!c || !c->configured || !name) return -1;
  const std::string key(name);
  for (auto& L : c->layers) {
    if (key == L.prefix + L.conv + ".weight") return L.off_w;
    if (key == L.prefix + L.conv + ".bias") return L.off_b;
    if (!L.bn.empty()) {
      if (key == L.prefix + L.bn + ".weight") return L.off_gamma;
      if (key == L.prefix + L.bn + ".bias") return L.off_beta;
    }
  }
  return -1;
}

int mgu_unet_load_weights(mgu_ctx* c, const mgu_tensor_desc* named, int n, void* hip_stream) {
  if (!c) return MGU_ERR_INVALID;
  if (!c->configured) return fail(c, MGU_ERR_STATE, "mgu_unet_configure must precede mgu_unet_load_weights");
  if (!named || n <= 0) return fail(c, MGU_ERR_INVALID, "empty state_dict");
  HIPCHK(c, hipSetDevice(c->device));
  hipStream_t s = (hipStream_t)hip_stream;
  std::map<std::string, const mgu_tensor_desc*> sd;
  for (int i = 0; i < n; ++i)
    if (named[i].name) sd[named[i].name] = &named[i];
  auto get = [&](const std::string& key, int64_t numel, const float** out) -> int {
    auto it = sd.find(key);
    if (it == sd.end()) return fail(c, MGU_ERR_INVALID, "state_dict is missing key '%s'", key.c_str());
    if (it->second->numel != numel)
      return fail(c, MGU_ERR_INVALID, "state_dict key '%s' has %lld elements, expected %lld", key.c_str(),
                  (long long)it->second->numel, (long long)numel);
    if (!it->second->ptr) return fail(c, MGU_ERR_INVALID, "state_dict key '%s' has a NULL pointer", key.c_str());
    *out = (const float*)it->second->ptr;
    return MGU_OK;
  };
  for (auto& L : c->layers) {
    const float *w, *b;
    const std::string cw = L.prefix + L.conv;
    int rc;
    if (L.convt) {
      if ((rc = get(cw + ".weight", (int64_t)L.Cin * L.Cout * 4, &w))) return rc;
      if ((rc = get(cw + ".bias", L.Cout, &b))) return rc;
      L.w_src = w, L.b_src = b;
    } else {
      if ((rc = get(cw + ".weight", (int64_t)L.Cout * L.Cin * L.KS * L.KS, &w))) return rc;
      if ((rc = get(cw + ".bias", L.Cout, &b))) return rc;
      L.w_src = w, L.b_src = b;
      if (!L.bn.empty()) {
        const float *g, *be, *rm, *rv;
        const std::string bn = L.prefix + L.bn;
        if ((rc = get(bn + ".weight", L.Cout, &g))) return rc;
        if ((rc = get(bn + ".bias", L.Cout, &be))) return rc;
        if ((rc = get(bn + ".running_mean", L.Cout, &rm))) return rc;
        if ((rc = get(bn + ".running_var", L.Cout, &rv))) return rc;
        L.gamma = g, L.beta = be, L.run_mean = const_cast<float*>(rm), L.run_var = const_cast<float*>(rv);
      }
    }
  }
  int rc = repack_weights(c, s);
  if (rc) return rc;
  c->loaded = true;
  return MGU_OK;
}

int mgu_unet_refresh_weights(mgu_ctx* c, void* hip_stream) {
  if (!c) return MGU_ERR_INVALID;
  if (!c->configured || !c->loaded) return fail(c, MGU_ERR_STATE, "mgu_unet_refresh_weights needs a preceding mgu_unet_load_weights");
  HIPCHK(c, hipSetDevice(c->device));
  return repack_weights(c, (hipStream_t)hip_stream);
}

int mgu_unet_workspace_bytes(mgu_ctx* c, int B, int H, int W, int training, size_t* out) {
  if (!c || !out) return MGU_ERR_INVALID;
  if (!c->configured) return fail(c, MGU_ERR_STATE, "not configured");
  *out = training ? train_ws_bytes(c, B, H, W) : plan_ws(c, B, H, W).total;
  return MGU_OK;
}

int mgu_unet_reserve(mgu_ctx* c, int B, int H, int W, int training) {
  size_t need = 0;
  int rc = mgu_unet_workspace_bytes(c, B, H, W, training, &need);
  if (rc) return rc;
  HIPCHK(c, hipSetDevice(c->device));
  return training ? ensure(c, &c->tws, &c->tws_bytes, need) : ensure(c, &c->ws, &c->ws_bytes, need);
}

}

int mgud::repack_weights(mgu_ctx* c, hipStream_t s) {
  std::vector<PackItem> items;
  for (auto& L : c->layers) {
    const float *w = L.w_src, *b = L.b_src;
    L.wxg_valid = false;
    if (L.convt) {
      L.wp_dirty = L.ctx3;
      if (!L.ctx3) items.push_back(pack_convt_panel(w, L.wp, c->dtype, L.Cin, L.Cout, L.Kp));
      if (L.ctb) items.push_back(pack_convt_bf16f(w, L.wu, L.Cin, L.Cout));
      if (L.ctx3) items.push_back(pack_convt_x3(w, L.wu, L.Cin, L.Cout, 0));
      items.push_back(pack_bias_tile(b, L.shift, L.Cout, 4));
      if (L.wxg && c->want_train && convt_x3_dgrad_layer(c->tn, L.Cin, L.Cout)) {
        items.push_back(pack_convt_x3(w, L.wxg, L.Cin, L.Cout, 1));
        L.wxg_valid = true;
      }
    } else {
      L.wp_dirty = true;
      if (L.wu) items.push_back(pack_wino(w, L.wu, L.Cout, L.Cin, L.Cp, 0, c->tn.wino_prec));
      L.wug_valid = false;
      if (L.wug && c->want_train && wino_dgrad_layer(c->tn, L.KS, rup(L.Cout, 4))) {
        items.push_back(pack_wino(w, L.wug, L.Cin, L.Cout, rup(L.Cout, 4), 1, c->tn.wino_prec));
        L.wug_valid = true;
      }
      const bool head_kernel = L.bn.empty() && c->ncls <= 4;
      if (!L.wu && !L.first && !head_kernel) {
        items.push_back(pack_conv_panel(w, L.wp, c->dtype, L.Cout, L.Cin, L.Cp, L.KS, L.Kp));
        L.wp_dirty = false;
      }
      if (L.wf) items.push_back(pack_first_w(w, L.wf, L.Cout, L.Cin));
      if (L.wfm && L.Cout == 32 && L.Cin <= 3) items.push_back(pack_first_mfma(w, L.wfm, L.Cout, L.Cin));
      if (!L.bn.empty()) c->fold_dirty = true;
      else items.push_back(pack_bias_tile(b, L.shift, L.Cout, 1));
      if (L.bn.empty() && L.wxg && c->want_train) {
        const int Cop = rup(L.Cout, 4);
        items.push_back(pack_dgrad_panel(w, L.wxg, L.Cout, L.Cin, Cop, L.KS, rup(L.KS * L.KS * Cop, 32)));
        L.wxg_valid = true;
      }
    }
  }
  std::vector<PackBatch> batches;
  for (size_t i0 = 0; i0 < items.size(); i0 += PACK_MAX) {
    PackBatch b;
    memset(&b, 0, sizeof b);
    b.n = (int)std::min<size_t>(PACK_MAX, items.size() - i0);
    for (int i = 0; i < b.n; ++i) b.it[i] = items[i0 + i];
    if (!pack_batch_prepare(b)) return fail(c, MGU_ERR_STATE, "internal: a weight form is not packable");
    batches.push_back(b);
  }
  const bool same = batches.size() == c->pack_host.size() &&
                    (batches.empty() || memcmp(batches.data(), c->pack_host.data(), batches.size() * sizeof(PackBatch)) == 0);
  if (!same) {
    if ((int)batches.size() > c->pack_dev_cap) {
      if (c->pack_dev) HIPCHK(c, hipFree(c->pack_dev));
      c->pack_dev = nullptr;
      HIPCHK(c, hipMalloc((void**)&c->pack_dev, batches.size() * sizeof(PackBatch)));
      c->pack_dev_cap = (int)batches.size();
    }
    HIPCHK(c, hipStreamSynchronize(s));
    HIPCHK(c, hipMemcpy(c->pack_dev, batches.data(), batches.size() * sizeof(PackBatch), hipMemcpyHostToDevice));
    c->pack_host = batches;
  }
  for (size_t k = 0; k < batches.size(); ++k) HIPCHK(c, launch_pack_batch(c->pack_dev + k, batches[k].total_blocks, s));
  return MGU_OK;
}

int mgud::run_layer(mgu_ctx* c, const Layer& L, const void* in_v, int ldin, int B, int H, int W, void* out_v, int ldout,
                    int coff, int relu, const float* scale, const float* shift, int Hout, int Wout, hipStream_t s,
                    void* pool, int ldpool, bool* pool_fused, double* stat_slots, bool* stat_fused, const WinoHead* head,
                    bool* head_fused) {
  IgemmDesc d = layer_desc(c, L, in_v, ldin, B, H, W, out_v, ldout, coff);
  if (head_fused) *head_fused = false;
  d.scale = scale, d.shift = shift, d.relu = relu, d.Hout = Hout, d.Wout = Wout;
  if (pool_fused) *pool_fused = false;
  if (stat_fused) *stat_fused = false;
  if (L.wfm && c->tn.first_mfma && ldin == L.Cp && first_mfma_applicable(c->dtype, L.Cin, L.Cp, L.Cout, ldout, coff, H, W)) {
    const double alg = 2.0 * d.M * 9.0 * L.Cin * L.Cout;
    ProfScope ps(c, s, "conv3x3_first_mfma_kernel", alg, 2.0 * d.M * 32.0 * 32.0 * (c->dtype == MGU_DTYPE_F32 ? 6.0 : 3.0), 1);
    HIPCHK(c, launch_first_mfma(c->dtype, in_v, L.wfm, scale, shift, out_v, B, H, W, ldout, coff, relu, s));
    return MGU_OK;
  }
  if (L.wf && ldin == L.Cp && first_conv_applicable(c->dtype, L.Cin, L.Cp, L.Cout, ldout, coff) &&
      (int64_t)B * H * W * std::max(ldout, 8) < (1ll << 31)) {
    ProfScope ps(c, s, "conv3x3_first_kernel", 2.0 * d.M * 9.0 * L.Cin * L.Cout, 0, -1);
    HIPCHK(c, launch_first_conv(c->dtype, in_v, L.wf, scale, shift, out_v, B, H, W, L.Cin, L.Cout, ldout, coff, relu, s));
    return MGU_OK;
  }
  ConvKernel k = pick_conv(d, c->dtype, head);
  if (stat_slots && conv_is_wino(k) && wino_grid_blocks(d) <= STAT_ROWS) {
    d.stat_slots = stat_slots;
    c->last_stat_rows = wino_grid_blocks(d);
    if (stat_fused) *stat_fused = true;
  }
  if (pool && conv_fuses_pool(k)) {
    d.pool = (float*)pool, d.ldpool = ldpool;
    if (pool_fused) *pool_fused = true;
  }
  if (d.stat_slots || d.pool) k = pick_conv(d, c->dtype, head);
  if (!conv_fuses_head(k)) head = nullptr;
  else if (head_fused) *head_fused = true;
  if (L.wp_dirty && conv_reads_panel(k)) {
    HIPCHK(c, launch_pack_one(L.convt ? pack_convt_panel(L.w_src, L.wp, c->dtype, L.Cin, L.Cout, L.Kp)
                                      : pack_conv_panel(L.w_src, L.wp, c->dtype, L.Cout, L.Cin, L.Cp, L.KS, L.Kp), s));
    L.wp_dirty = false;
  }
  double alg = L.convt ? 2.0 * d.M * (double)L.Cin * L.Cout * 4.0 : 2.0 * d.M * (double)L.KS * L.KS * L.Cin * L.Cout;
  if (head) alg += 2.0 * d.M * (double)L.Cout * head->ncls;
  const ConvCost cost = conv_cost(k, d);
  ProfScope ps(c, s, conv_kernel_name(k, d), alg, cost.mfma, cost.pipe);
  HIPCHK(c, launch_conv(d, k, c->dtype, s, head));
  return MGU_OK;
}

static int run_conv(mgu_ctx* c, const Layer& L, const void* in, int ldin, int B, int H, int W, void* out, int ldout,
                    int coff, int relu, int Hout, int Wout, hipStream_t s, void* pool = nullptr, int ldpool = 0,
                    bool* pool_fused = nullptr, const WinoHead* head = nullptr, bool* head_fused = nullptr) {
  return run_layer(c, L, in, ldin, B, H, W, out, ldout, coff, relu, L.bn.empty() ? nullptr : L.scale, L.shift, Hout, Wout, s,
                   pool, ldpool, pool_fused, nullptr, nullptr, head, head_fused);
}

extern "C" {

int mgu_unet_forward(mgu_ctx* c, const void* x_dev, int B, int H, int W, int64_t xs_n, int64_t xs_c, int64_t xs_h,
                     int64_t xs_w, void* logits_dev, void* const* cat_dev, void* const* feat_dev, int training,
                     void* hip_stream) {
  if (!c) return MGU_ERR_INVALID;
  if (!c->configured || !c->loaded) return fail(c, MGU_ERR_STATE, "configure + load_weights must precede forward");
  if (!x_dev || !logits_dev || !cat_dev || !feat_dev) return fail(c, MGU_ERR_INVALID, "NULL buffer");
  const int depth = c->depth;
  if (B < 1 || H < (1 << depth) || W < (1 << depth))
    return fail(c, MGU_ERR_INVALID, "input %dx%dx%d too small for depth %d", B, H, W, depth);
  if ((int64_t)B * H * W >= (1ll << 31)) return fail(c, MGU_ERR_INVALID, "B*H*W must be < 2^31");
  for (int i = 0; i < depth; ++i)
    if (!cat_dev[i] || !feat_dev[i]) return fail(c, MGU_ERR_INVALID, "NULL cat/feat buffer %d", i);
  HIPCHK(c, hipSetDevice(c->device));
  hipStream_t s = (hipStream_t)hip_stream;
  if (training && c->dtype != MGU_DTYPE_F32)
    return fail(c, MGU_ERR_STATE, "training runs in fp32 only (bf16 storage is an inference mode)");
  if (training) {
    int rc = unet_forward_train(c, (const float*)x_dev, xs_n, xs_c, xs_h, xs_w, B, H, W, (float*)logits_dev, cat_dev, feat_dev, s);
    if (rc == MGU_OK && c->pm_out) {
      ProfScope ps(c, s, "patch_mean_kernel", 0, 0, -1);
      HIPCHK(c, launch_patch_mean(feat_dev[0], 0, (float*)c->pm_out, B, H, W, c->feat, c->pm_patch, s));
      c->pm_out = nullptr;
    }
    return rc;
  }
  const WsPlan plan = plan_ws(c, B, H, W);
  int rc = ensure(c, &c->ws, &c->ws_bytes, plan.total);
  if (rc) return rc;
  const Layer& F = c->layers[c->head];
  WinoHead head_args{};
  bool head_done = false;
  const bool head_wanted = c->pm_out && F.w_src && F.b_src && wino_head_layer(c->tn, c->dtype, F.Cin, c->ncls, c->pm_patch, B, H, W);
  if (head_wanted) {
    if ((rc = ensure(c, &c->pmws, &c->pmws_bytes, wino_head_psum_bytes(B, H, W)))) return rc;
    head_args = WinoHead{F.w_src, F.b_src, (float*)logits_dev, (float*)c->pmws, c->ncls, (int)wino_head_psum_bytes(B, H, W)};
  }
  if (c->fold_dirty) {
    for (auto& L : c->layers)
      if (!L.bn.empty()) HIPCHK(c, launch_bn_fold(L.b_src, L.gamma, L.beta, L.run_mean, L.run_var, 1e-5f, L.scale, L.shift, L.Cout, s));
    c->fold_dirty = false;
  }
  char* ws = (char*)c->ws;
  const size_t es = c->dtype == MGU_DTYPE_BF16 ? 2 : 4;
  void* xin = ws + plan.xin;
  void* tmp = ws + plan.tmp;
  void* bott = ws + plan.bott;
  std::vector<int> hs, wsz;
  level_dims(H, W, depth, hs, wsz);

  if (c->prof) {
    for (auto& e : c->ev_total)
      if (!e) HIPCHK(c, hipEventCreate(&e));
    HIPCHK(c, hipEventRecord(c->ev_total[0], s));
  }

  for (const Block& b : c->enc) {
    const int i = b.level;
    if (2 * hs[i + 1] != hs[i] || 2 * wsz[i + 1] != wsz[i])
      HIPCHK(c, hipMemsetAsync(cat_dev[i], 0, (size_t)B * hs[i] * wsz[i] * 2 * c->layers[b.conv2].Cout * es, s));
  }

  const Layer& L0 = c->layers[c->enc[0].conv1];
  const bool first_direct = L0.wfm && c->tn.first_mfma && first_mfma_applicable(c->dtype, L0.Cin, L0.Cp, L0.Cout, c->feat, 0, H, W) &&
                            (int64_t)B * H * W < (1ll << 31);
  if (!first_direct) HIPCHK(c, launch_pack_input((const float*)x_dev, xin, c->dtype, B, c->in_ch, c->Cp0, H, W, xs_n, xs_c, xs_h, xs_w, s));

  const void* cur = xin;
  int cur_ld = c->Cp0;
  for (const Block& b : c->enc) {
    const int i = b.level, C = c->layers[b.conv1].Cout;
    if (&b == &c->enc.front() && first_direct) {
      if (c->fold_dirty) return fail(c, MGU_ERR_STATE, "internal: eval scale/shift not folded");
      const double alg = 2.0 * B * H * W * 9.0 * L0.Cin * L0.Cout;
      ProfScope ps(c, s, "conv3x3_first_mfma_kernel", alg, 2.0 * B * H * W * 32.0 * 32.0 * (c->dtype == MGU_DTYPE_F32 ? 6.0 : 3.0), 1);
      HIPCHK(c, launch_first_mfma_direct(c->dtype, (const float*)x_dev, xs_n, xs_c, xs_h, xs_w, c->in_ch, L0.wfm, L0.bn.empty() ? nullptr : L0.scale,
                                         L0.shift, tmp, B, H, W, C, 0, 1, s));
    } else if ((rc = run_conv(c, c->layers[b.conv1], cur, cur_ld, B, hs[i], wsz[i], tmp, C, 0, 1, 0, 0, s))) return rc;
    void* pooled = ws + plan.pooled[i];
    bool fused = false;
    if ((rc = run_conv(c, c->layers[b.conv2], tmp, C, B, hs[i], wsz[i], cat_dev[i], 2 * C, 0, 1, 0, 0, s, pooled, C, &fused))) return rc;
    if (!fused) HIPCHK(c, launch_maxpool2(cat_dev[i], 2 * C, pooled, c->dtype, B, hs[i], wsz[i], C, s));
    cur = pooled;
    cur_ld = C;
  }
  {
    const Block& b = c->bott;
    const int i = b.level, C = c->layers[b.conv1].Cout;
    if ((rc = run_conv(c, c->layers[b.conv1], cur, cur_ld, B, hs[i], wsz[i], tmp, C, 0, 1, 0, 0, s))) return rc;
    if ((rc = run_conv(c, c->layers[b.conv2], tmp, C, B, hs[i], wsz[i], bott, C, 0, 1, 0, 0, s))) return rc;
    cur = bott;
    cur_ld = C;
  }
  for (const Block& b : c->dec) {
    const int i = b.level, C = c->layers[b.conv1].Cout;
    const bool last = head_wanted && i == 0;
    if ((rc = run_conv(c, c->layers[b.up], cur, cur_ld, B, hs[i + 1], wsz[i + 1], cat_dev[i], 2 * C, C, 0, hs[i], wsz[i], s)))
      return rc;
    if ((rc = run_conv(c, c->layers[b.conv1], cat_dev[i], 2 * C, B, hs[i], wsz[i], tmp, C, 0, 1, 0, 0, s))) return rc;
    if ((rc = run_conv(c, c->layers[b.conv2], tmp, C, B, hs[i], wsz[i], feat_dev[i], C, 0, 1, 0, 0, s, nullptr, 0, nullptr,
                       last ? &head_args : nullptr, last ? &head_done : nullptr)))
      return rc;
    cur = feat_dev[i];
    cur_ld = C;
  }
  {
    const int pm_dtype = c->dtype;
    if (head_done) {
      ProfScope ps(c, s, "patch_sum_combine_kernel", 0, 0, -1);
      HIPCHK(c, launch_patch_sum_combine((const float*)c->pmws, (float*)c->pm_out, B * (H / 16) * (W / 16), s));
      c->pm_out = nullptr;
    } else if (c->pm_out && F.w_src && F.b_src && patch_mean_head_fusable(pm_dtype, F.Cin, c->ncls) && F.Cin <= 256) {
      ProfScope ps(c, s, "patch_mean_kernel (1x1 head + patch means)", 2.0 * B * H * W * F.Cin * c->ncls, 0, -1);
      HIPCHK(c, launch_patch_mean(cur, pm_dtype, (float*)c->pm_out, B, H, W, F.Cin, c->pm_patch, s, F.w_src, F.b_src,
                                  (float*)logits_dev, c->ncls));
      c->pm_out = nullptr;
    } else if (c->ncls <= 4 && F.w_src && F.b_src) {
      ProfScope ps(c, s, "conv1x1_head_kernel", 2.0 * B * H * W * F.Cin * c->ncls, 0, -1);
      HIPCHK(c, launch_conv1x1_head(cur, c->dtype, cur_ld, F.Cin, F.w_src, F.b_src, (float*)logits_dev, c->ncls, c->ncls,
                                    (int64_t)B * H * W, s));
    } else if ((rc = run_conv(c, F, cur, cur_ld, B, H, W, logits_dev, c->ncls, 0, 0, 0, 0, s))) {
      return rc;
    }
  }
  if (c->pm_out) {
    ProfScope ps(c, s, "patch_mean_kernel", 0, 0, -1);
    HIPCHK(c, launch_patch_mean(cur, c->dtype, (float*)c->pm_out, B, H, W, F.Cin, c->pm_patch, s));
    c->pm_out = nullptr;
  }
  if (c->prof) HIPCHK(c, hipEventRecord(c->ev_total[1], s));
  return MGU_OK;
}

int mgu_unet_request_patch_mean(mgu_ctx* c, int patch, void* out_dev) {
  if (!c) return MGU_ERR_INVALID;
  if (!c->configured) return fail(c, MGU_ERR_STATE, "not configured");
  if (!out_dev) {
    c->pm_out = nullptr;
    return MGU_OK;
  }
  if (patch < 1) return fail(c, MGU_ERR_INVALID, "bad patch_mean request");
  const int C = c->layers[c->head].Cin, vec = c->dtype == MGU_DTYPE_BF16 ? 8 : 4;
  if ((C % vec) || C > 256) return fail(c, MGU_ERR_INVALID, "patch means need init_features %% %d == 0 and <= 256 (got %d)", vec, C);
  c->pm_patch = patch;
  c->pm_out = out_dev;
  return MGU_OK;
}

struct mgu_conv_weights {
  Layer L;
};

static Layer block_layer(int Cin, int Cout, int ksize, bool convt) {
  Layer L;
  L.Cin = L.Cp = Cin, L.Cout = Cout, L.KS = ksize, L.convt = convt;
  L.K = ksize * ksize * Cin, L.Kp = rup(L.K, 32), L.N = convt ? 4 * Cout : Cout, L.Np = rup(L.N, 128);
  return L;
}

static int conv2d_launch(mgu_ctx* c, const Layer& L, const void* in_dev, int B, int H, int W, const void* bias_dev, const void* scale_dev,
                         const void* shift_dev, int relu, void* out_dev, int ld_out, int c_off, hipStream_t s) {
  IgemmDesc d = layer_desc(c, L, in_dev, L.Cin, B, H, W, out_dev, ld_out, c_off);
  d.relu = relu;
  if (scale_dev && shift_dev) {
    d.scale = (const float*)scale_dev;
    d.shift = (const float*)shift_dev;
  } else if (bias_dev) {
    HIPCHK(c, launch_pack_one(pack_bias_tile((const float*)bias_dev, L.shift, L.Cout, 1), s));
    d.shift = L.shift;
  }
  const ConvKernel k = pick_conv(d, 0);
  ProfScope ps(c, s, conv_kernel_name(k, d));
  HIPCHK(c, launch_conv(d, k, 0, s));
  return MGU_OK;
}

int mgu_conv2d_prepare(mgu_ctx* c, const void* w_dev, int Cout, int Cin, int ksize, mgu_conv_weights** out, void* hip_stream) {
  if (!c) return MGU_ERR_INVALID;
  if (!w_dev || !out || Cout < 1 || (ksize != 1 && ksize != 3)) return fail(c, MGU_ERR_INVALID, "bad conv2d_prepare args (ksize must be 1 or 3)");
  if (Cin < 4 || (Cin & 3)) return fail(c, MGU_ERR_INVALID, "conv2d needs Cin %% 4 == 0 (got %d)", Cin);
  HIPCHK(c, hipSetDevice(c->device));
  hipStream_t s = (hipStream_t)hip_stream;
  mgu_conv_weights* p = new mgu_conv_weights();
  Layer& L = p->L;
  L = block_layer(Cin, Cout, ksize, false);
  const bool wino = wino_layer(c->tn, ksize, Cin);
  const size_t panel = (size_t)L.Np * L.Kp, total = panel + L.Np + (wino ? wino_u_floats(Cout, Cin) : 0);
  hipError_t e = hipMalloc((void**)&L.wp, total * sizeof(float));
  if (e != hipSuccess) {
    delete p;
    return fail(c, MGU_ERR_NOMEM, "hipMalloc(%zu) failed: %s", total * sizeof(float), hipGetErrorString(e));
  }
  L.shift = L.wp + panel;
  e = hipMemsetAsync(L.wp, 0, (panel + L.Np) * sizeof(float), s);
  if (e == hipSuccess) e = launch_pack_one(pack_conv_panel((const float*)w_dev, L.wp, 0, Cout, Cin, Cin, ksize, L.Kp), s);
  if (e == hipSuccess && wino) {
    L.wu = L.shift + L.Np;
    e = launch_pack_one(pack_wino((const float*)w_dev, L.wu, Cout, Cin, Cin, 0, c->tn.wino_prec), s);
  }
  if (e != hipSuccess) {
    (void)hipFree(L.wp);
    delete p;
    return fail(c, MGU_ERR_HIP, "conv2d_prepare: %s", hipGetErrorString(e));
  }
  *out = p;
  return MGU_OK;
}

void mgu_conv2d_release(mgu_ctx* c, mgu_conv_weights* p) {
  if (!p) return;
  if (c) (void)hipSetDevice(c->device);
  (void)hipDeviceSynchronize();
  if (p->L.wp) (void)hipFree(p->L.wp);
  delete p;
}

int mgu_conv2d_prepared_nhwc(mgu_ctx* c, const mgu_conv_weights* p, const void* in_dev, int B, int H, int W, const void* bias_dev,
                             const void* scale_dev, const void* shift_dev, int relu, void* out_dev, int ld_out, int c_off,
                             void* hip_stream) {
  if (!c) return MGU_ERR_INVALID;
  if (!p || !in_dev || !out_dev || B < 1 || H < 1 || W < 1) return fail(c, MGU_ERR_INVALID, "bad conv2d args");
  if (ld_out < c_off + p->L.Cout) return fail(c, MGU_ERR_INVALID, "ld_out %d < c_off %d + Cout %d", ld_out, c_off, p->L.Cout);
  if ((int64_t)B * H * W >= (1ll << 31)) return fail(c, MGU_ERR_INVALID, "B*H*W must be < 2^31");
  HIPCHK(c, hipSetDevice(c->device));
  return conv2d_launch(c, p->L, in_dev, B, H, W, bias_dev, scale_dev, shift_dev, relu, out_dev, ld_out, c_off, (hipStream_t)hip_stream);
}

int mgu_conv2d_nhwc(mgu_ctx* c, const void* in_dev, int B, int H, int W, int Cin, const void* w_dev, const void* bias_dev,
                    const void* scale_dev, const void* shift_dev, int Cout, int ksize, int relu, void* out_dev,
                    int ld_out, int c_off, void* hip_stream) {
  if (!c) return MGU_ERR_INVALID;
  if (!in_dev || !w_dev || !out_dev || B < 1 || H < 1 || W < 1 || Cout < 1 || (ksize != 1 && ksize != 3))
    return fail(c, MGU_ERR_INVALID, "bad conv2d args (ksize must be 1 or 3)");
  if (Cin < 4 || (Cin & 3)) return fail(c, MGU_ERR_INVALID, "conv2d needs Cin %% 4 == 0 (got %d)", Cin);
  if (ld_out < c_off + Cout) return fail(c, MGU_ERR_INVALID, "ld_out %d < c_off %d + Cout %d", ld_out, c_off, Cout);
  if ((int64_t)B * H * W >= (1ll << 31)) return fail(c, MGU_ERR_INVALID, "B*H*W must be < 2^31");
  HIPCHK(c, hipSetDevice(c->device));
  hipStream_t s = (hipStream_t)hip_stream;
  Layer L = block_layer(Cin, Cout, ksize, false);
  const size_t need = ((size_t)L.Np * L.Kp + 2 * (size_t)L.Np) * sizeof(float);
  int rc = ensure(c, &c->gws, &c->gws_bytes, need);
  if (rc) return rc;
  L.wp = (float*)c->gws;
  L.shift = L.wp + (size_t)L.Np * L.Kp + L.Np;
  HIPCHK(c, hipMemsetAsync(c->gws, 0, need, s));
  HIPCHK(c, launch_pack_one(pack_conv_panel((const float*)w_dev, L.wp, 0, Cout, Cin, Cin, ksize, L.Kp), s));
  if (wino_layer(c->tn, ksize, Cin)) {
    if ((rc = ensure(c, &c->wuws, &c->wuws_bytes, wino_u_floats(Cout, Cin) * sizeof(float)))) return rc;
    L.wu = (float*)c->wuws;
    HIPCHK(c, launch_pack_one(pack_wino((const float*)w_dev, L.wu, Cout, Cin, Cin, 0, c->tn.wino_prec), s));
  }
  return conv2d_launch(c, L, in_dev, B, H, W, bias_dev, scale_dev, shift_dev, relu, out_dev, ld_out, c_off, s);
}

int mgu_conv_transpose2x2_nhwc(mgu_ctx* c, const void* in_dev, int B, int H, int W, int Cin, const void* w_dev,
                               const void* bias_dev, int Cout, void* out_dev, int ld_out, int c_off, void* hip_stream) {
  if (!c) return MGU_ERR_INVALID;
  if (!in_dev || !w_dev || !out_dev || B < 1 || H < 1 || W < 1 || Cout < 1) return fail(c, MGU_ERR_INVALID, "bad convT args");
  if (Cin < 4 || (Cin & 3)) return fail(c, MGU_ERR_INVALID, "convT needs Cin %% 4 == 0 (got %d)", Cin);
  if (ld_out < c_off + Cout) return fail(c, MGU_ERR_INVALID, "ld_out %d < c_off %d + Cout %d", ld_out, c_off, Cout);
  if ((int64_t)B * H * W * 4 >= (1ll << 31)) return fail(c, MGU_ERR_INVALID, "4*B*H*W must be < 2^31");
  HIPCHK(c, hipSetDevice(c->device));
  hipStream_t s = (hipStream_t)hip_stream;
  Layer U = block_layer(Cin, Cout, 1, true);
  const bool x3_shape = convt_x3_layer(c->tn, Cin, Cout);
  const size_t panel = (size_t)U.Np * U.Kp + 2 * (size_t)U.Np;
  int rc = ensure(c, &c->gws, &c->gws_bytes, (panel + (x3_shape ? convt_x3_floats(Cin, Cout) : 0)) * sizeof(float));
  if (rc) return rc;
  U.wp = (float*)c->gws;
  U.shift = U.wp + (size_t)U.Np * U.Kp + U.Np;
  U.wu = x3_shape ? U.wp + panel : nullptr;
  HIPCHK(c, hipMemsetAsync(c->gws, 0, panel * sizeof(float), s));
  HIPCHK(c, launch_pack_one(pack_convt_panel((const float*)w_dev, U.wp, 0, Cin, Cout, U.Kp), s));
  IgemmDesc d = layer_desc(c, U, in_dev, Cin, B, H, W, out_dev, ld_out, c_off);
  d.Hout = 2 * H, d.Wout = 2 * W;
  if (bias_dev) {
    HIPCHK(c, launch_pack_one(pack_bias_tile((const float*)bias_dev, U.shift, Cout, 4), s));
    d.shift = U.shift;
  }
  const ConvKernel k = pick_conv(d, 0);
  if (k == ConvKernel::ConvtX3) HIPCHK(c, launch_pack_one(pack_convt_x3((const float*)w_dev, U.wu, Cin, Cout, 0), s));
  ProfScope ps(c, s, conv_kernel_name(k, d));
  HIPCHK(c, launch_conv(d, k, 0, s));
  return MGU_OK;
}

int mgu_maxpool2x2_nhwc(mgu_ctx* c, const void* in_dev, int ld_in, int B, int H, int W, int Cc, void* out_dev,
                        void* hip_stream) {
  if (!c) return MGU_ERR_INVALID;
  if (!in_dev || !out_dev || B < 1 || H < 2 || W < 2 || Cc < 4 || (Cc & 3) || ld_in < Cc || (ld_in & 3))
    return fail(c, MGU_ERR_INVALID, "bad maxpool args (C and ld_in must be multiples of 4, H,W >= 2)");
  HIPCHK(c, hipSetDevice(c->device));
  HIPCHK(c, launch_maxpool2(in_dev, ld_in, out_dev, 0, B, H, W, Cc, (hipStream_t)hip_stream));
  return MGU_OK;
}

int mgu_argmax_classes(mgu_ctx* c, const void* logits_dev, int64_t npix, int num_classes, int64_t* pred_dev,
                       void* hip_stream) {
  if (!c || !logits_dev || !pred_dev || num_classes < 1 || npix < 0) return fail(c, MGU_ERR_INVALID, "bad argmax args");
  HIPCHK(c, hipSetDevice(c->device));
  HIPCHK(c, launch_argmax((const float*)logits_dev, npix, num_classes, pred_dev, (hipStream_t)hip_stream));
  return MGU_OK;
}

int mgu_patch_mean(mgu_ctx* c, const void* feat_dev, int feat_dtype, int B, int H, int W, int C, int patch, void* out_dev,
                   void* hip_stream) {
  if (!c || !feat_dev || !out_dev || B < 1 || H < 1 || W < 1 || patch < 1)
    return fail(c, MGU_ERR_INVALID, "bad patch_mean args");
  if (feat_dtype != MGU_DTYPE_F32 && feat_dtype != MGU_DTYPE_BF16) return fail(c, MGU_ERR_INVALID, "unknown dtype %d", feat_dtype);
  const int vec = feat_dtype == MGU_DTYPE_BF16 ? 8 : 4;
  if ((C % vec) || C < vec || C > 256)
    return fail(c, MGU_ERR_INVALID, "patch_mean needs C %% %d == 0 and C <= 256 (got %d)", vec, C);
  HIPCHK(c, hipSetDevice(c->device));
  HIPCHK(c, launch_patch_mean(feat_dev, feat_dtype, (float*)out_dev, B, H, W, C, patch, (hipStream_t)hip_stream));
  return MGU_OK;
}

static double net_flops(const mgu_ctx* c, int B, int H, int W, bool mfma) {
  std::vector<int> hs, wsz;
  level_dims(H, W, c->depth, hs, wsz);
  double fl = 0;
  for (const Layer& L : c->layers) {
    const int h = hs[L.level], w = wsz[L.level];
    if (mfma && L.wino) fl += 2.0 * ((h + 1) / 2) * ((w + 1) / 2) * 16.0 * L.Cp * L.Cout;
    else fl += 2.0 * h * w * L.KS * L.KS * L.Cin * L.Cout * (L.convt ? 4.0 : 1.0);
  }
  return fl * B;
}

double mgu_unet_flops(mgu_ctx* c, int B, int H, int W) { return c && c->configured ? net_flops(c, B, H, W, false) : -1.0; }

double mgu_unet_mfma_flops(mgu_ctx* c, int B, int H, int W) { return c && c->configured ? net_flops(c, B, H, W, true) : -1.0; }

int mgu_profile_enable(mgu_ctx* c, int on) {
  if (!c) return MGU_ERR_INVALID;
  c->prof = on != 0;
  c->ev_used = 0;
  return MGU_OK;
}

int mgu_profile_read_kernels(mgu_ctx* c, mgu_kernel_stat* out, int cap, int* n_out) {
  if (!c || !n_out || (cap > 0 && !out)) return MGU_ERR_INVALID;
  int n = 0;
  for (int i = 0; i < c->ev_used; ++i) {
    float ms = 0;
    HIPCHK(c, hipEventSynchronize(c->ev[2 * i + 1]));
    HIPCHK(c, hipEventElapsedTime(&ms, c->ev[2 * i], c->ev[2 * i + 1]));
    const mgu_ctx::ProfRec& r = c->prec[i];
    int k = 0;
    while (k < n && strcmp(out[k].name, r.name) != 0) ++k;
    if (k == n) {
      if (n == cap) continue;
      out[n].name = r.name, out[n].ms = 0, out[n].flops_alg = 0, out[n].flops_mfma = 0, out[n].launches = 0, out[n].pipe = r.pipe;
      ++n;
    }
    out[k].ms += ms, out[k].flops_alg += r.alg, out[k].flops_mfma += r.mfma, out[k].launches += 1;
  }
  *n_out = n;
  c->ev_used = 0;
  return MGU_OK;
}

int mgu_profile_read(mgu_ctx* c, double* conv_ms, int* conv_launches, double* total_ms) {
  if (!c) return MGU_ERR_INVALID;
  if (c->ev_used == 0 || !c->ev_total[1]) return fail(c, MGU_ERR_STATE, "no profiled forward to read");
  HIPCHK(c, hipEventSynchronize(c->ev_total[1]));
  double sum = 0;
  for (int i = 0; i < c->ev_used; ++i) {
    float ms = 0;
    HIPCHK(c, hipEventSynchronize(c->ev[2 * i + 1]));
    HIPCHK(c, hipEventElapsedTime(&ms, c->ev[2 * i], c->ev[2 * i + 1]));
    sum += ms;
  }
  float tot = 0;
  HIPCHK(c, hipEventElapsedTime(&tot, c->ev_total[0], c->ev_total[1]));
  if (conv_ms) *conv_ms = sum;
  if (conv_launches) *conv_launches = c->ev_used;
  if (total_ms) *total_ms = tot;
  return MGU_OK;
}

}
```

mingraph-unet_amd/csrc/pack.hip:

```cpp
#include "common.h"

#include <algorithm>

namespace mgu {

enum { PACK_WINO, PACK_FIRST_W, PACK_CONVT_X3, PACK_BIAS_TILE, PACK_DGRAD_PANEL, PACK_FIRST_MFMA, PACK_CONV_PANEL, PACK_CONVT_PANEL,
       PACK_CONVT_BF16F, PACK_CONVT_DGRAD_PANEL };


__device__ __forceinline__ void pack_wino_w_body(const float* __restrict__ w, float* __restrict__ U, int Cout, int Cin, int Cp, int Np,
                                                 int dgrad, int prec, unsigned vblock, unsigned vgrid) {
  if (prec == 1) {
    const int nC = Cp >> 4;
    const int64_t total8 = (int64_t)Np * (Cp >> 3);
    for (int64_t idx = vblock * (int64_t)blockDim.x + threadIdx.x; idx < total8; idx += (int64_t)vgrid * blockDim.x) {
      const int lane = (int)(idx & 63);
      const int64_t grp = idx >> 6;
      const int c16 = (int)(grp % nC), ntile = (int)(grp / nC);
      const int n = ntile * 32 + (lane & 31), c0 = c16 * 16 + (lane >> 5) * 8;
      float g[8][3][3];
#pragma unroll
      for (int e = 0; e < 8; ++e)
#pragma unroll
        for (int u = 0; u < 3; ++u)
#pragma unroll
          for (int v = 0; v < 3; ++v) {
            const int c = c0 + e;
            float x = 0.f;
            if (n < Cout && c < Cin)
              x = dgrad ? w[(((int64_t)c * Cout + n) * 3 + (2 - u)) * 3 + (2 - v)] : w[(((int64_t)n * Cin + c) * 3 + u) * 3 + v];
            g[e][u][v] = x;
          }
      u32x4* dst = reinterpret_cast<u32x4*>(U) + ((int64_t)ntile * nC + c16) * 16 * 192 + lane;
#pragma unroll
      for (int i = 0; i < 4; ++i)
#pragma unroll
        for (int j = 0; j < 4; ++j) {
          unsigned short p0[8], p1[8], p2[8];
#pragma unroll
          for (int e = 0; e < 8; ++e) {
            float t3[3];
#pragma unroll
            for (int v = 0; v < 3; ++v)
              t3[v] = i == 0 ? g[e][0][v] : i == 3 ? g[e][2][v] : 0.5f * (g[e][0][v] + (i == 1 ? g[e][1][v] : -g[e][1][v]) + g[e][2][v]);
            const float uv = j == 0 ? t3[0] : j == 3 ? t3[2] : 0.5f * (t3[0] + (j == 1 ? t3[1] : -t3[1]) + t3[2]);
            const unsigned b0 = __float_as_uint(uv) & 0xffff0000u;
            const float r1 = uv - __uint_as_float(b0);
            const unsigned b1 = __float_as_uint(r1) & 0xffff0000u;
            const float r2 = r1 - __uint_as_float(b1);
            p0[e] = (unsigned short)(b0 >> 16), p1[e] = (unsigned short)(b1 >> 16), p2[e] = (unsigned short)(__float_as_uint(r2) >> 16);
          }
          u32x4 q0, q1, q2;
#pragma unroll
          for (int e = 0; e < 4; ++e) {
            q0[e] = (unsigned)p0[2 * e] | ((unsigned)p0[2 * e + 1] << 16);
            q1[e] = (unsigned)p1[2 * e] | ((unsigned)p1[2 * e + 1] << 16);
            q2[e] = (unsigned)p2[2 * e] | ((unsigned)p2[2 * e + 1] << 16);
          }
          u32x4* q = dst + (i * 4 + j) * 192;
          q[0] = q0, q[64] = q1, q[128] = q2;
        }
    }
    return;
  }
  const int64_t total = (int64_t)Np * Cp;
  for (int64_t idx = vblock * (int64_t)blockDim.x + threadIdx.x; idx < total; idx += (int64_t)vgrid * blockDim.x) {
    const int c = (int)(idx % Cp), n = (int)(idx / Cp);
    float g[3][3];
#pragma unroll
    for (int u = 0; u < 3; ++u)
#pragma unroll
      for (int v = 0; v < 3; ++v) {
        float x = 0.f;
        if (n < Cout && c < Cin) {
          x = dgrad ? w[(((int64_t)c * Cout + n) * 3 + (2 - u)) * 3 + (2 - v)] : w[(((int64_t)n * Cin + c) * 3 + u) * 3 + v];
        }
        g[u][v] = x;
      }
    float t[4][3];
#pragma unroll
    for (int v = 0; v < 3; ++v) {
      t[0][v] = g[0][v];
      t[1][v] = 0.5f * (g[0][v] + g[1][v] + g[2][v]);
      t[2][v] = 0.5f * (g[0][v] - g[1][v] + g[2][v]);
      t[3][v] = g[2][v];
    }
    float u[4][4];
#pragma unroll
    for (int i = 0; i < 4; ++i) {
      u[i][0] = t[i][0];
      u[i][1] = 0.5f * (t[i][0] + t[i][1] + t[i][2]);
      u[i][2] = 0.5f * (t[i][0] - t[i][1] + t[i][2]);
      u[i][3] = t[i][2];
    }
    float* dst = U + (((int64_t)(n >> 5) * (Cp >> 3) + (c >> 3)) * 16) * 256 + ((((c >> 2) & 1) * 32 + (n & 31)) * 4 + (c & 3));
#pragma unroll
    for (int i = 0; i < 4; ++i)
#pragma unroll
      for (int j = 0; j < 4; ++j) dst[(i * 4 + j) * 256] = u[i][j];
  }
}

__device__ __forceinline__ void pack_first_w_body(const float* __restrict__ w, float* __restrict__ wf, int Cout, int Cin, unsigned vblock,
                                                  unsigned vgrid) {
  const int total = 9 * 4 * Cout;
  for (int i = (int)(vblock * blockDim.x + threadIdx.x); i < total; i += (int)(vgrid * blockDim.x)) {
    const int co = i % Cout, c = (i / Cout) % 4, tap = i / (4 * Cout);
    wf[i] = c < Cin ? w[((int64_t)co * Cin + c) * 9 + tap] : 0.f;
  }
}

__device__ __forceinline__ void pack_bias_tile_body(const float* __restrict__ bias, float* __restrict__ shift, int C, int reps, unsigned vblock,
                                                    unsigned vgrid) {
  for (int i = (int)(vblock * blockDim.x + threadIdx.x); i < C * reps; i += (int)(vgrid * blockDim.x)) shift[i] = bias[i % C];
}

__device__ __forceinline__ void pack_convt_x3_body(const float* __restrict__ w, uint16_t* __restrict__ Wx, int Cin, int Cout, int dgrad,
                                                   unsigned vblock, unsigned vgrid) {
  const int K = dgrad ? 4 * Cout : Cin;
  const int64_t total = (int64_t)Cin * Cout * 4;
  const int ksteps = K >> 4;
  for (int64_t idx = vblock * (int64_t)blockDim.x + threadIdx.x; idx < total; idx += (int64_t)vgrid * blockDim.x) {
    const int k = (int)(idx % K), n = (int)(idx / K);
    const int q = dgrad ? k / Cout : n / Cout;
    const int co = dgrad ? k - q * Cout : n - q * Cout;
    const int ci = dgrad ? n : k;
    const float x = w[(((int64_t)ci * Cout + co) * 2 + (q >> 1)) * 2 + (q & 1)];
    const unsigned b0 = __float_as_uint(x) & 0xffff0000u;
    const float r1 = x - __uint_as_float(b0);
    const unsigned b1 = __float_as_uint(r1) & 0xffff0000u;
    const float r2 = r1 - __uint_as_float(b1);
    const int lane = ((k >> 3) & 1) * 32 + (n & 31);
    uint16_t* dst = Wx + (((((int64_t)(n >> 7) * ksteps + (k >> 4)) * 4 + ((n >> 5) & 3)) * 3) * 64 + lane) * 8 + (k & 7);
    dst[0] = (uint16_t)(b0 >> 16);
    dst[512] = (uint16_t)(b1 >> 16);
    dst[1024] = (uint16_t)(__float_as_uint(r2) >> 16);
  }
}

__device__ __forceinline__ void pack_first_mfma_body(const float* __restrict__ w, uint16_t* __restrict__ wfm, int Cout, int Cin, unsigned vblock,
                                                     unsigned vgrid) {
  for (int i = (int)(vblock * blockDim.x + threadIdx.x); i < 2 * 64 * 8; i += (int)(vgrid * blockDim.x)) {
    const int e = i & 7, lane = (i >> 3) & 63, s = i >> 9;
    const int co = lane & 31, h = lane >> 5, j = 8 * s + e;
    const int tap = 5 * h + j / 3, ch = j % 3;
    float x = 0.f;
    if (j < 15 && tap < 9 && ch < Cin && co < Cout) x = w[((int64_t)co * Cin + ch) * 9 + tap];
    const unsigned b0 = __float_as_uint(x) & 0xffff0000u;
    const float r1 = x - __uint_as_float(b0);
    const unsigned b1 = __float_as_uint(r1) & 0xffff0000u;
    const float r2 = r1 - __uint_as_float(b1);
    uint16_t* dst = wfm + ((size_t)(s * 3) * 64 + lane) * 8 + e;
    dst[0] = (uint16_t)(b0 >> 16);
    dst[512] = (uint16_t)(b1 >> 16);
    dst[1024] = (uint16_t)(__float_as_uint(r2) >> 16);
  }
}

__device__ __forceinline__ void pack_dgrad_w_body(const float* __restrict__ w, float* __restrict__ wp, int Cout, int Cin, int Cop, int KS, int Kp,
                                                  unsigned vblock, unsigned vgrid) {
  const int64_t total = (int64_t)Cin * Kp;
  for (int64_t i = vblock * (int64_t)blockDim.x + threadIdx.x; i < total; i += (int64_t)vgrid * blockDim.x) {
    const int ci = (int)(i / Kp), k = (int)(i - (int64_t)ci * Kp);
    const int tap = k / Cop, co = k - tap * Cop;
    float v = 0.f;
    if (tap < KS * KS && co < Cout) v = w[((int64_t)co * Cin + ci) * KS * KS + (KS * KS - 1 - tap)];
    wp[i] = v;
  }
}

template <typename T>
__device__ __forceinline__ void pack_conv_w_body(const float* __restrict__ w, T* __restrict__ wp, int Cout, int Cin, int Cp, int KS, int Kp,
                                                 unsigned vblock, unsigned vgrid) {
  const int64_t total = (int64_t)Cout * Kp;
  for (int64_t i = vblock * (int64_t)blockDim.x + threadIdx.x; i < total; i += (int64_t)vgrid * blockDim.x) {
    const int n = (int)(i / Kp), k = (int)(i - (int64_t)n * Kp);
    const int tap = k / Cp, c = k - tap * Cp;
    float v = 0.f;
    if (tap < KS * KS && c < Cin) v = w[((int64_t)n * Cin + c) * KS * KS + tap];
    wp[i] = (T)v;
  }
}

template <typename T>
__device__ __forceinline__ void pack_convt_w_body(const float* __restrict__ w, T* __restrict__ wp, int Cin, int Cout, int Kp, unsigned vblock,
                                                  unsigned vgrid) {
  const int64_t total = (int64_t)4 * Cout * Kp;
  for (int64_t i = vblock * (int64_t)blockDim.x + threadIdx.x; i < total; i += (int64_t)vgrid * blockDim.x) {
    const int n = (int)(i / Kp), k = (int)(i - (int64_t)n * Kp);
    const int q = n / Cout, co = n - q * Cout;
    wp[i] = (T)((k < Cin) ? w[((int64_t)k * Cout + co) * 4 + q] : 0.f);
  }
}

__device__ __forceinline__ void pack_convt_bf16f_body(const float* __restrict__ w, __bf16* __restrict__ Wf, int Cin, int Cout, unsigned vblock,
                                                      unsigned vgrid) {
  const int64_t total = (int64_t)Cin * Cout * 4;
  const int ksteps = Cin >> 4;
  for (int64_t idx = vblock * (int64_t)blockDim.x + threadIdx.x; idx < total; idx += (int64_t)vgrid * blockDim.x) {
    const int k = (int)(idx % Cin), n = (int)(idx / Cin);
    const int q = n / Cout, co = n - q * Cout;
    const float x = w[(((int64_t)k * Cout + co) * 2 + (q >> 1)) * 2 + (q & 1)];
    const int lane = ((k >> 3) & 1) * 32 + (n & 31);
    Wf[(((((int64_t)(n >> 7) * ksteps + (k >> 4)) * 4 + ((n >> 5) & 3))) * 64 + lane) * 8 + (k & 7)] = (__bf16)x;
  }
}

__device__ __forceinline__ void pack_convt_dgrad_w_body(const float* __restrict__ w, float* __restrict__ wp, int Cin, int Cout, int Kp,
                                                        unsigned vblock, unsigned vgrid) {
  const int64_t total = (int64_t)Cin * Kp;
  for (int64_t i = vblock * (int64_t)blockDim.x + threadIdx.x; i < total; i += (int64_t)vgrid * blockDim.x) {
    const int ci = (int)(i / Kp), k = (int)(i - (int64_t)ci * Kp);
    const int q = k / Cout, co = k - q * Cout;
    wp[i] = (q < 4) ? w[((int64_t)ci * Cout + co) * 4 + q] : 0.f;
  }
}

size_t wino_u_floats(int Cout, int Cp) { return (size_t)((Cout + 63) / 64 * 64) * Cp * 24; }
size_t convt_x3_floats(int Cin, int Cout) { return (size_t)Cin * Cout * 6; }
size_t convt_x3_dgrad_floats(int Cin, int Cout) { return (size_t)((Cin + 127) / 128 * 128) * Cout * 6; }
size_t convt_bf16f_floats(int Cin, int Cout) { return (size_t)Cin * Cout * 2; }
size_t first_mfma_floats() { return 2 * 3 * 64 * 4; }

static PackItem item(int kind, const float* w, void* out, int Cout, int Cin, int Cp = 0, int Np = 0, int dgrad = 0, int mode = 0) {
  return PackItem{w, (float*)out, Cout, Cin, Cp, Np, dgrad, 0u, kind, mode};
}
PackItem pack_wino(const float* w, float* U, int Cout, int Cin, int Cp, int dgrad, int prec) {
  return item(PACK_WINO, w, U, Cout, Cin, Cp, (Cout + 63) / 64 * 64, dgrad, prec);
}
PackItem pack_first_w(const float* w, float* wf, int Cout, int Cin) { return item(PACK_FIRST_W, w, wf, Cout, Cin); }
PackItem pack_first_mfma(const float* w, float* wfm, int Cout, int Cin) { return item(PACK_FIRST_MFMA, w, wfm, Cout, Cin); }
PackItem pack_convt_x3(const float* w, float* Wx, int Cin, int Cout, int dgrad) { return item(PACK_CONVT_X3, w, Wx, Cout, Cin, 0, 0, dgrad); }
PackItem pack_bias_tile(const float* bias, float* shift, int C, int reps) { return item(PACK_BIAS_TILE, bias, shift, C, reps); }
PackItem pack_dgrad_panel(const float* w, float* wp, int Cout, int Cin, int Cop, int KS, int Kp) {
  return item(PACK_DGRAD_PANEL, w, wp, Cout, Cin, Cop, Kp, KS);
}
PackItem pack_conv_panel(const float* w, void* wp, int dtype, int Cout, int Cin, int Cp, int KS, int Kp) {
  return item(PACK_CONV_PANEL, w, wp, Cout, Cin, Cp, Kp, KS, dtype);
}
PackItem pack_convt_panel(const float* w, void* wp, int dtype, int Cin, int Cout, int Kp) {
  return item(PACK_CONVT_PANEL, w, wp, Cout, Cin, 0, Kp, 0, dtype);
}
PackItem pack_convt_bf16f(const float* w, float* Wf, int Cin, int Cout) { return item(PACK_CONVT_BF16F, w, Wf, Cout, Cin); }
PackItem pack_convt_dgrad_panel(const float* w, float* wp, int Cin, int Cout, int Kp) {
  return item(PACK_CONVT_DGRAD_PANEL, w, wp, Cout, Cin, 0, Kp);
}

__device__ __forceinline__ void pack_item(const PackItem& t, unsigned vblock, unsigned vgrid) {
  switch (t.kind) {
    case PACK_WINO: pack_wino_w_body(t.w, t.U, t.Cout, t.Cin, t.Cp, t.Np, t.dgrad, t.mode, vblock, vgrid); break;
    case PACK_FIRST_W: pack_first_w_body(t.w, t.U, t.Cout, t.Cin, vblock, vgrid); break;
    case PACK_FIRST_MFMA: pack_first_mfma_body(t.w, reinterpret_cast<uint16_t*>(t.U), t.Cout, t.Cin, vblock, vgrid); break;
    case PACK_CONVT_X3: pack_convt_x3_body(t.w, reinterpret_cast<uint16_t*>(t.U), t.Cin, t.Cout, t.dgrad, vblock, vgrid); break;
    case PACK_BIAS_TILE: pack_bias_tile_body(t.w, t.U, t.Cout, t.Cin, vblock, vgrid); break;
    case PACK_DGRAD_PANEL: pack_dgrad_w_body(t.w, t.U, t.Cout, t.Cin, t.Cp, t.dgrad, t.Np, vblock, vgrid); break;
    case PACK_CONV_PANEL:
      if (t.mode == 0) pack_conv_w_body(t.w, t.U, t.Cout, t.Cin, t.Cp, t.dgrad, t.Np, vblock, vgrid);
      else pack_conv_w_body(t.w, reinterpret_cast<__bf16*>(t.U), t.Cout, t.Cin, t.Cp, t.dgrad, t.Np, vblock, vgrid);
      break;
    case PACK_CONVT_PANEL:
      if (t.mode == 0) pack_convt_w_body(t.w, t.U, t.Cin, t.Cout, t.Np, vblock, vgrid);
      else pack_convt_w_body(t.w, reinterpret_cast<__bf16*>(t.U), t.Cin, t.Cout, t.Np, vblock, vgrid);
      break;
    case PACK_CONVT_BF16F: pack_convt_bf16f_body(t.w, reinterpret_cast<__bf16*>(t.U), t.Cin, t.Cout, vblock, vgrid); break;
    case PACK_CONVT_DGRAD_PANEL: pack_convt_dgrad_w_body(t.w, t.U, t.Cin, t.Cout, t.Np, vblock, vgrid); break;
    default: break;
  }
}

static unsigned pack_item_blocks(const PackItem& t) {
  int64_t work;
  switch (t.kind) {
    case PACK_WINO:
      if ((t.mode != 0 && t.mode != 1) || (t.Cp & (t.mode ? 15 : 7))) return 0;
      work = (int64_t)t.Np * t.Cp / (t.mode ? 8 : 1);
      break;
    case PACK_FIRST_W: work = 9 * 4 * (int64_t)t.Cout; break;
    case PACK_FIRST_MFMA: work = 2 * 64 * 8; break;
    case PACK_CONVT_X3:
      if ((t.Cin & (t.dgrad ? 63 : 15)) || (t.Cout & 31)) return 0;
      work = (int64_t)t.Cin * t.Cout * 4;
      break;
    case PACK_BIAS_TILE: work = (int64_t)t.Cout * t.Cin; break;
    case PACK_DGRAD_PANEL: work = (int64_t)t.Cin * t.Np; break;
    case PACK_CONV_PANEL: work = (int64_t)t.Cout * t.Np; break;
    case PACK_CONVT_PANEL: work = (int64_t)4 * t.Cout * t.Np; break;
    case PACK_CONVT_BF16F:
      if ((t.Cin & 63) || (t.Cout & 31)) return 0;
      work = (int64_t)t.Cin * t.Cout * 4;
      break;
    case PACK_CONVT_DGRAD_PANEL: work = (int64_t)t.Cin * t.Np; break;
    default: return 0;
  }
  return (unsigned)std::max<int64_t>(1, std::min<int64_t>(2048, (work + 255) / 256));
}

__global__ void pack_batch_kernel(const PackBatch* __restrict__ bp) {
  const PackBatch& b = *bp;
  int i = 0;
  while (i + 1 < b.n && blockIdx.x >= b.it[i + 1].blk0) ++i;
  const PackItem& t = b.it[i];
  pack_item(t, blockIdx.x - t.blk0, (i + 1 < b.n ? b.it[i + 1].blk0 : b.total_blocks) - t.blk0);
}

__global__ void pack_one_kernel(const PackItem it) { pack_item(it, blockIdx.x, gridDim.x); }

bool pack_batch_prepare(PackBatch& b) {
  unsigned blk = 0;
  for (int i = 0; i < b.n; ++i) {
    const unsigned blocks = pack_item_blocks(b.it[i]);
    if (!blocks) return false;
    b.it[i].blk0 = blk;
    blk += blocks;
  }
  b.total_blocks = blk;
  return true;
}

hipError_t launch_pack_batch(const PackBatch* batch_dev, unsigned total_blocks, hipStream_t s) {
  if (total_blocks == 0) return hipSuccess;
  hipLaunchKernelGGL(pack_batch_kernel, dim3(total_blocks), dim3(256), 0, s, batch_dev);
  return hipGetLastError();
}

hipError_t launch_pack_one(const PackItem& it, hipStream_t s) {
  const unsigned blocks = pack_item_blocks(it);
  if (!blocks) return hipErrorInvalidValue;
  hipLaunchKernelGGL(pack_one_kernel, dim3(blocks), dim3(256), 0, s, it);
  return hipGetLastError();
}

}
```

Baseline: 806.0.

## Add 16x16x32 bf16 MFMA variant of split-bf16x3 transposed-conv kernel

Adds a new ConvTranspose 2x2 kernel that uses the 16x16x32 bf16 MFMA instruction instead of the 32x32x16 form. It packs a second weight copy in a matching fragment layout and picks this kernel by default when the grid has at least 64 tiles. The goal is better MFMA throughput and scheduling, using explicit sched_group_barriers to interleave MFMA with LDS reads. The cost is extra weight storage and packing work, plus different register and LDS access patterns.

```diff
diff --git a/mingraph-unet_amd/csrc/common.h b/mingraph-unet_amd/csrc/common.h
--- a/mingraph-unet_amd/csrc/common.h
+++ b/mingraph-unet_amd/csrc/common.h
@@ -19,6 +19,7 @@
   bool use_wino = true;
   int wino_prec = 1;
   bool convt_frag = true;
+  int convt_k32 = -1;
   bool wino_cp = true;
   int wino_ppb_cap = 32;
   bool wgrad_halo = true;
@@ -86,6 +87,7 @@
   HaloF32, HaloBf16Np8, HaloBf16Np4,
   TilesF32, TilesBf16,
   ConvtX3, ConvtBf16f, ConvtX3Dgrad,
+  ConvtX3K32,
 };
 ConvKernel pick_conv(const IgemmDesc& d, int dtype, const WinoHead* head = nullptr);
 hipError_t launch_conv(const IgemmDesc& d, ConvKernel k, int dtype, hipStream_t s, const WinoHead* head = nullptr);
@@ -104,11 +106,13 @@
   return conv_is_wino(k) || (k >= ConvKernel::HaloF32 && k <= ConvKernel::HaloBf16Np4);
 }
 inline bool conv_reads_panel(ConvKernel k) {
-  return !conv_is_wino(k) && k != ConvKernel::ConvtX3 && k != ConvKernel::ConvtBf16f && k != ConvKernel::ConvtX3Dgrad;
+  return !conv_is_wino(k) && k != ConvKernel::ConvtX3 && k != ConvKernel::ConvtBf16f && k != ConvKernel::ConvtX3Dgrad &&
+         k != ConvKernel::ConvtX3K32;
 }
 bool wino_layer(const Tuning& t, int KS, int Cp);
 bool wino_dgrad_layer(const Tuning& t, int KS, int Cop);
 bool convt_x3_layer(const Tuning& t, int Cin, int Cout);
+bool convt_x3_k32_layer(const Tuning& t, int Cin, int Cout);
 bool convt_x3_dgrad_layer(const Tuning& t, int Cin, int Cout);
 bool convt_bf16f_layer(const Tuning& t, int Cin, int Cout);
 bool wino_head_layer(const Tuning& t, int dtype, int Cin, int ncls, int patch, int B, int H, int W);
@@ -119,6 +123,7 @@
 WinoPlan wino_plan(const IgemmDesc& d);
 int wino_grid_blocks(const IgemmDesc& d);
 hipError_t launch_convt_x3(const IgemmDesc& d, hipStream_t s);
+hipError_t launch_convt_x3_k32(const IgemmDesc& d, hipStream_t s);
 hipError_t launch_convt_bf16f(const IgemmDesc& d, hipStream_t s);
 hipError_t launch_convt_x3_dgrad(const IgemmDesc& d, hipStream_t s);
 bool first_mfma_applicable(int dtype, int Cin, int Cp, int Cout, int ldout, int coff, int64_t H, int64_t W);
@@ -146,7 +151,7 @@
 PackItem pack_wino(const float* w, float* U, int Cout, int Cin, int Cp, int dgrad, int prec);
 PackItem pack_first_w(const float* w, float* wf, int Cout, int Cin);
 PackItem pack_first_mfma(const float* w, float* wfm, int Cout, int Cin);
-PackItem pack_convt_x3(const float* w, float* Wx, int Cin, int Cout, int dgrad);
+PackItem pack_convt_x3(const float* w, float* Wx, int Cin, int Cout, int dgrad, int k32 = 0);
 PackItem pack_bias_tile(const float* bias, float* shift, int C, int reps);
 PackItem pack_dgrad_panel(const float* w, float* wp, int Cout, int Cin, int Cop, int KS, int Kp);
 PackItem pack_conv_panel(const float* w, void* wp, int dtype, int Cout, int Cin, int Cp, int KS, int Kp);
diff --git a/mingraph-unet_amd/csrc/convt_x3.hip b/mingraph-unet_amd/csrc/convt_x3.hip
--- a/mingraph-unet_amd/csrc/convt_x3.hip
+++ b/mingraph-unet_amd/csrc/convt_x3.hip
@@ -191,6 +191,158 @@
   else store_tile(std::true_type{});
 }
 
+__global__ __launch_bounds__(256, 2) void convt2x2_x3_k32_kernel(const float* __restrict__ in, const int ldin, const uint16_t* __restrict__ Wk,
+                                                                 const float* __restrict__ shift, float* __restrict__ out, const int M,
+                                                                 const int H, const int W, const int Cin, const int Cout, const int ldout,
+                                                                 const int coff, const int Hout, const int Wout, const int ntn,
+                                                                 const int nblocks) {
+  constexpr int AP = 40, ABUF = 3 * 128 * AP;
+  __shared__ __attribute__((aligned(16))) uint16_t As[2 * ABUF];
+  __shared__ int rowoff[128];
+  const int chunk = gridDim.x >> 3;
+  const int lb = (blockIdx.x & 7) * chunk + (blockIdx.x >> 3);
+  if (lb >= nblocks) return;
+  const int nt = lb % ntn, mt = lb / ntn;
+  const int tid = threadIdx.x, lane = tid & 63, wave = tid >> 6;
+  const int wm = wave >> 1, wn = wave & 1, lc = lane & 15, lg = lane >> 4;
+  const int bm0 = mt * 128;
+  const int HW = H * W;
+  long long pix0;
+  {
+    const int img = bm0 / HW, rem = bm0 - img * HW, y = rem / W;
+    pix0 = ((long long)img * Hout + 2 * y) * Wout + 2 * (rem - y * W);
+  }
+  if (tid < 128) {
+    const int m = bm0 + tid;
+    int off = 0;
+    if (m < M) {
+      const int img = m / HW, rem = m - img * HW, y = rem / W, x = rem - y * W;
+      off = (int)((((long long)img * Hout + 2 * y) * Wout + 2 * x - pix0) * ldout);
+    }
+    rowoff[tid] = off;
+  }
+
+  const int arow = tid >> 3, ach = (tid & 7) * 4;
+  const float* aptr[4];
+#pragma unroll
+  for (int j = 0; j < 4; ++j) aptr[j] = in + (size_t)min(bm0 + j * 32 + arow, M - 1) * ldin + ach;
+  const int nk = Cin >> 5;
+  f32x4 areg[2][4];
+  auto load_a = [&](int s, auto set_t) {
+    constexpr int set = decltype(set_t)::value;
+#pragma unroll
+    for (int j = 0; j < 4; ++j) areg[set][j] = *reinterpret_cast<const f32x4*>(aptr[j] + s * 32);
+  };
+  auto store_a = [&](int buf, auto set_t) {
+    constexpr int set = decltype(set_t)::value;
+    uint16_t* const base = As + buf * ABUF + arow * AP + ach;
+#pragma unroll
+    for (int j = 0; j < 4; ++j) {
+      unsigned p[3][2];
+      split3_pack(areg[set][j][0], areg[set][j][1], p[0][0], p[1][0], p[2][0]);
+      split3_pack(areg[set][j][2], areg[set][j][3], p[0][1], p[1][1], p[2][1]);
+#pragma unroll
+      for (int q = 0; q < 3; ++q) *reinterpret_cast<uint2*>(base + (q * 128 + j * 32) * AP) = uint2{p[q][0], p[q][1]};
+    }
+  };
+
+  const u32x4* const bp = reinterpret_cast<const u32x4*>(Wk) + ((size_t)nt * nk * 24 + wn * 12) * 64 + lane;
+  u32x4 br[2][6];
+  auto load_b = [&](int kk, auto buf_t) {
+    constexpr int buf = decltype(buf_t)::value;
+    const size_t f0 = (size_t)(kk >> 1) * 24 + (kk & 1) * 6;
+#pragma unroll
+    for (int f = 0; f < 6; ++f) br[buf][f] = bp[(f0 + f) * 64];
+  };
+
+  f32x4 acc[4][4];
+#pragma unroll
+  for (int mi = 0; mi < 4; ++mi)
+#pragma unroll
+    for (int nj = 0; nj < 4; ++nj)
+#pragma unroll
+      for (int r = 0; r < 4; ++r) acc[mi][nj][r] = 0.f;
+
+  const int aoff = (wm * 64 + lc) * AP + lg * 8;
+  auto half_step = [&](int buf, auto hh_t) {
+    constexpr int hh = decltype(hh_t)::value;
+#pragma unroll
+    for (int mi = 0; mi < 4; ++mi) {
+      u32x4 pa[3];
+#pragma unroll
+      for (int q = 0; q < 3; ++q) pa[q] = *reinterpret_cast<const u32x4*>(As + buf * ABUF + (q * 128 + mi * 16) * AP + aoff);
+#pragma unroll
+      for (int ni = 0; ni < 2; ++ni) {
+        f32x4 t = acc[mi][hh * 2 + ni];
+        t = mfma_bf16_k32(pa[2], br[hh][ni * 3 + 0], t);
+        t = mfma_bf16_k32(pa[0], br[hh][ni * 3 + 2], t);
+        t = mfma_bf16_k32(pa[1], br[hh][ni * 3 + 1], t);
+        t = mfma_bf16_k32(pa[1], br[hh][ni * 3 + 0], t);
+        t = mfma_bf16_k32(pa[0], br[hh][ni * 3 + 1], t);
+        t = mfma_bf16_k32(pa[0], br[hh][ni * 3 + 0], t);
+        acc[mi][hh * 2 + ni] = t;
+      }
+    }
+  };
+  using B0 = std::integral_constant<int, 0>;
+  using B1 = std::integral_constant<int, 1>;
+  const int nkk = 2 * nk;
+  load_a(0, B0{});
+  load_a(min(1, nk - 1), B1{});
+  load_b(0, B0{});
+  store_a(0, B0{});
+  lds_barrier();
+  auto step = [&](int s, int buf, auto set_t) {
+    load_a(min(s + 2, nk - 1), std::integral_constant<int, 1 - decltype(set_t)::value>{});
+    load_b(min(2 * s + 1, nkk - 1), B1{});
+    __builtin_amdgcn_sched_barrier(0);
+    half_step(buf, B0{});
+    load_b(min(2 * s + 2, nkk - 1), B0{});
+    __builtin_amdgcn_sched_barrier(0);
+    half_step(buf, B1{});
+    store_a(buf ^ 1, set_t);
+#pragma unroll
+    for (int k = 0; k < 48; ++k) {
+      __builtin_amdgcn_sched_group_barrier(0x008, 1, 0);
+      __builtin_amdgcn_sched_group_barrier(0x002, 2, 0);
+    }
+    __builtin_amdgcn_sched_group_barrier(0x200, 12, 0);
+    __builtin_amdgcn_sched_barrier(0);
+    lds_barrier();
+  };
+  int s = 0;
+  for (; s + 1 < nk; s += 2) {
+    step(s, 0, B1{});
+    step(s + 1, 1, B0{});
+  }
+  if (s < nk) step(s, 0, B1{});
+
+  float* const tile_out = out + (size_t)pix0 * ldout + coff;
+  const bool full_m = bm0 + 128 <= M;
+  auto store_tile = [&](auto guarded_t) {
+    constexpr bool GUARDED = decltype(guarded_t)::value;
+#pragma unroll
+    for (int nj = 0; nj < 4; ++nj) {
+      const int n = nt * 128 + wn * 64 + nj * 16 + lc;
+      const int q = n / Cout;
+      const int ncol = ((q >> 1) * Wout + (q & 1)) * ldout + (n - q * Cout);
+      const float sh = shift ? shift[n] : 0.f;
+#pragma unroll
+      for (int mi = 0; mi < 4; ++mi)
+#pragma unroll
+        for (int r = 0; r < 4; ++r) {
+          const int rrow = wm * 64 + mi * 16 + 4 * lg + r;
+          const unsigned idx = (unsigned)(rowoff[rrow] + ncol);
+          const float v = acc[mi][nj][r] + sh;
+          if (!GUARDED) tile_out[idx] = v;
+          else if (bm0 + rrow < M) tile_out[idx] = v;
+        }
+    }
+  };
+  if (full_m) store_tile(std::false_type{});
+  else store_tile(std::true_type{});
+}
+
 }
 
 hipError_t launch_convt_x3_dgrad(const IgemmDesc& d, hipStream_t s) {
@@ -216,4 +368,13 @@
   return hipGetLastError();
 }
 
-}
+hipError_t launch_convt_x3_k32(const IgemmDesc& d, hipStream_t s) {
+  const int mtiles = (d.M + 127) / 128, ntn = d.N / 128;
+  const int nb = mtiles * ntn;
+  const int chunk = (nb + 7) / 8;
+  hipLaunchKernelGGL(convt2x2_x3_k32_kernel, dim3(chunk * 8), dim3(256), 0, s, d.in, d.ldin, reinterpret_cast<const uint16_t*>(d.wu + convt_x3_floats(d.Cp, d.ct_cout)), d.shift,
+                     d.out, d.M, d.H, d.W, d.Cp, d.ct_cout, d.ldout, d.coff, d.Hout, d.Wout, ntn, nb);
+  return hipGetLastError();
+}
+
+}
diff --git a/mingraph-unet_amd/csrc/device.h b/mingraph-unet_amd/csrc/device.h
--- a/mingraph-unet_amd/csrc/device.h
+++ b/mingraph-unet_amd/csrc/device.h
@@ -48,6 +48,9 @@
 
 __device__ __forceinline__ f32x16 mfma_bf16(const u32x4 a, const u32x4 b, const f32x16 c) {
   return __builtin_amdgcn_mfma_f32_32x32x16_bf16(__builtin_bit_cast(bf16x8, a), __builtin_bit_cast(bf16x8, b), c, 0, 0, 0);
+}
+__device__ __forceinline__ f32x4 mfma_bf16_k32(const u32x4 a, const u32x4 b, const f32x4 c) {
+  return __builtin_amdgcn_mfma_f32_16x16x32_bf16(__builtin_bit_cast(bf16x8, a), __builtin_bit_cast(bf16x8, b), c, 0, 0, 0);
 }
 
 template <int I, int N, class F>
diff --git a/mingraph-unet_amd/csrc/igemm.hip b/mingraph-unet_amd/csrc/igemm.hip
--- a/mingraph-unet_amd/csrc/igemm.hip
+++ b/mingraph-unet_amd/csrc/igemm.hip
@@ -625,6 +625,7 @@
 bool wino_layer(const Tuning& t, int KS, int Cp) { return t.use_wino && KS == 3 && Cp % 16 == 0; }
 bool wino_dgrad_layer(const Tuning& t, int KS, int Cop) { return t.wino_dgrad && wino_layer(t, KS, Cop); }
 bool convt_x3_layer(const Tuning& t, int Cin, int Cout) { return t.wino_prec != 0 && t.convt_frag && Cin % 32 == 0 && Cout % 32 == 0; }
+bool convt_x3_k32_layer(const Tuning& t, int Cin, int Cout) { return convt_x3_layer(t, Cin, Cout) && t.convt_k32 != 0; }
 bool convt_x3_dgrad_layer(const Tuning& t, int Cin, int Cout) {
   return t.wino_prec != 0 && t.convt_dgrad_x3 && Cin % 64 == 0 && Cout % 32 == 0;
 }
@@ -667,6 +668,12 @@
 static bool convt_x3_applicable(const IgemmDesc& d) {
   return convt_x3_layer(tun(d), d.Cp, d.ct_cout) && d.wu && d.KS == 1 && d.K == d.Cp && d.N == 4 * d.ct_cout && (d.ldin & 3) == 0 &&
          !d.scale && !d.relu && !d.split_n && (9l * 128 + 8l * d.Wout) * d.ldout < (1l << 31);
+}
+
+static bool convt_x3_k32_applicable(const IgemmDesc& d) {
+  const Tuning& t = tun(d);
+  return convt_x3_applicable(d) && convt_x3_k32_layer(t, d.Cp, d.ct_cout) &&
+         (t.convt_k32 > 0 || ((long)d.H * d.W + 127) / 128 * (d.N / 128) >= 64);
 }
 
 static bool convt_bf16f_applicable(const IgemmDesc& d) {
@@ -689,7 +696,7 @@
     if (np) return np == 8 ? K::HaloBf16Np8 : K::HaloBf16Np4;
     return d.KS == 3 || d.KS == 1 ? K::TilesBf16 : K::None;
   }
-  if (d.out_mode == 1) return d.KS != 1 ? K::None : convt_x3_applicable(d) ? K::ConvtX3 : K::TilesF32;
+  if (d.out_mode == 1) return d.KS != 1 ? K::None : convt_x3_k32_applicable(d) ? K::ConvtX3K32 : convt_x3_applicable(d) ? K::ConvtX3 : K::TilesF32;
   if (convt_x3_dgrad_applicable(d)) return K::ConvtX3Dgrad;
   if (wino_applicable(d)) {
     const Tuning& t = tun(d);
@@ -722,6 +729,7 @@
     case ConvKernel::HaloBf16Np8: case ConvKernel::HaloBf16Np4: return "conv3x3_halo_kernel<bf16>";
     case ConvKernel::TilesBf16: return d.out_mode == 1 ? "igemm_kernel<bf16> (ConvTranspose)" : "igemm_kernel<bf16>";
     case ConvKernel::ConvtX3: return "convt2x2_x3_kernel";
+    case ConvKernel::ConvtX3K32: return "convt2x2_x3_kernel<16x16x32>";
     case ConvKernel::ConvtBf16f: return "convt2x2_bf16_kernel";
     case ConvKernel::ConvtX3Dgrad: return "convt2x2_x3_kernel<dgrad>";
     case ConvKernel::TilesF32: case ConvKernel::None: break;
@@ -747,7 +755,7 @@
   switch (k) {
     case ConvKernel::WinoF32Wide: case ConvKernel::WinoF32Narrow:
       return {2.0 * (d.M / (d.H * d.W)) * ((d.H + 1) / 2) * ((d.W + 1) / 2) * 16.0 * d.Cp * d.N, 0};
-    case ConvKernel::ConvtX3: case ConvKernel::ConvtX3Dgrad: return {6.0 * direct, 1};
+    case ConvKernel::ConvtX3: case ConvKernel::ConvtX3K32: case ConvKernel::ConvtX3Dgrad: return {6.0 * direct, 1};
     case ConvKernel::HaloBf16Np8: case ConvKernel::HaloBf16Np4: case ConvKernel::TilesBf16: case ConvKernel::ConvtBf16f: return {direct, 1};
     case ConvKernel::HaloF32: case ConvKernel::TilesF32: case ConvKernel::None: return {direct, 0};
     default:
@@ -783,6 +791,7 @@
       if (d.KS == 3) return launch_tiles<__bf16, 3, 0>(d, s);
       return launch_tiles<__bf16, 1, 0>(d, s);
     case ConvKernel::ConvtX3: return launch_convt_x3(d, s);
+    case ConvKernel::ConvtX3K32: return launch_convt_x3_k32(d, s);
     case ConvKernel::ConvtBf16f: return launch_convt_bf16f(d, s);
     case ConvKernel::ConvtX3Dgrad: return launch_convt_x3_dgrad(d, s);
     case ConvKernel::None: break;
diff --git a/mingraph-unet_amd/csrc/mgunet_api.hip b/mingraph-unet_amd/csrc/mgunet_api.hip
--- a/mingraph-unet_amd/csrc/mgunet_api.hip
+++ b/mingraph-unet_amd/csrc/mgunet_api.hip
@@ -45,7 +45,7 @@
   form(L.shift, (size_t)L.Np);
   if (L.wino) form(L.wu, wino_u_floats(L.Cout, L.Cp));
   if (L.wino && rup(L.Cout, 4) % 16 == 0) form(L.wug, wino_u_floats(L.Cin, rup(L.Cout, 4)));
-  if (L.ctx3) form(L.wu, convt_x3_floats(L.Cin, L.Cout));
+  if (L.ctx3) form(L.wu, convt_x3_floats(L.Cin, L.Cout) * (convt_x3_k32_layer(c->tn, L.Cin, L.Cout) ? 2 : 1));
   if (L.ctb) form(L.wu, convt_bf16f_floats(L.Cin, L.Cout));
   if (L.ctx3) form(L.wxg, convt_x3_dgrad_floats(L.Cin, L.Cout));
   if (dtype == MGU_DTYPE_F32 && !L.convt && L.bn.empty())
@@ -86,6 +86,7 @@
   t.wino_prec = num("MGU_WINO_PREC", t.wino_prec) ? 1 : 0;
   t.wino_cp = !flag("MGU_NO_WINO_CP");
   t.convt_frag = !flag("MGU_NO_CONVT_FRAG");
+  t.convt_k32 = num("MGU_CONVT_K32", -1);
   t.wino_ppb_cap = std::max(1, num("MGU_WINO_PPB_CAP", 32));
   t.wgrad_halo = !flag("MGU_NO_WGRAD_HALO");
   t.wino_wgrad = !flag("MGU_NO_WINO_WGRAD");
@@ -315,6 +316,8 @@
       if (!L.ctx3) items.push_back(pack_convt_panel(w, L.wp, c->dtype, L.Cin, L.Cout, L.Kp));
       if (L.ctb) items.push_back(pack_convt_bf16f(w, L.wu, L.Cin, L.Cout));
       if (L.ctx3) items.push_back(pack_convt_x3(w, L.wu, L.Cin, L.Cout, 0));
+      if (L.ctx3 && convt_x3_k32_layer(c->tn, L.Cin, L.Cout))
+        items.push_back(pack_convt_x3(w, L.wu + convt_x3_floats(L.Cin, L.Cout), L.Cin, L.Cout, 0, 1));
       items.push_back(pack_bias_tile(b, L.shift, L.Cout, 4));
       if (L.wxg && c->want_train && convt_x3_dgrad_layer(c->tn, L.Cin, L.Cout)) {
         items.push_back(pack_convt_x3(w, L.wxg, L.Cin, L.Cout, 1));
@@ -691,7 +694,7 @@
   Layer U = block_layer(Cin, Cout, 1, true);
   const bool x3_shape = convt_x3_layer(c->tn, Cin, Cout);
   const size_t panel = (size_t)U.Np * U.Kp + 2 * (size_t)U.Np;
-  int rc = ensure(c, &c->gws, &c->gws_bytes, (panel + (x3_shape ? convt_x3_floats(Cin, Cout) : 0)) * sizeof(float));
+  int rc = ensure(c, &c->gws, &c->gws_bytes, (panel + (x3_shape ? 2 * convt_x3_floats(Cin, Cout) : 0)) * sizeof(float));
   if (rc) return rc;
   U.wp = (float*)c->gws;
   U.shift = U.wp + (size_t)U.Np * U.Kp + U.Np;
@@ -706,6 +709,8 @@
   }
   const ConvKernel k = pick_conv(d, 0);
   if (k == ConvKernel::ConvtX3) HIPCHK(c, launch_pack_one(pack_convt_x3((const float*)w_dev, U.wu, Cin, Cout, 0), s));
+  if (k == ConvKernel::ConvtX3K32)
+    HIPCHK(c, launch_pack_one(pack_convt_x3((const float*)w_dev, U.wu + convt_x3_floats(Cin, Cout), Cin, Cout, 0, 1), s));
   ProfScope ps(c, s, conv_kernel_name(k, d));
   HIPCHK(c, launch_conv(d, k, 0, s));
   return MGU_OK;
diff --git a/mingraph-unet_amd/csrc/pack.hip b/mingraph-unet_amd/csrc/pack.hip
--- a/mingraph-unet_amd/csrc/pack.hip
+++ b/mingraph-unet_amd/csrc/pack.hip
@@ -115,7 +115,7 @@
   for (int i = (int)(vblock * blockDim.x + threadIdx.x); i < C * reps; i += (int)(vgrid * blockDim.x)) shift[i] = bias[i % C];
 }
 
-__device__ __forceinline__ void pack_convt_x3_body(const float* __restrict__ w, uint16_t* __restrict__ Wx, int Cin, int Cout, int dgrad,
+__device__ __forceinline__ void pack_convt_x3_body(const float* __restrict__ w, uint16_t* __restrict__ Wx, int Cin, int Cout, int dgrad, int k32,
                                                    unsigned vblock, unsigned vgrid) {
   const int K = dgrad ? 4 * Cout : Cin;
   const int64_t total = (int64_t)Cin * Cout * 4;
@@ -130,8 +130,10 @@
     const float r1 = x - __uint_as_float(b0);
     const unsigned b1 = __float_as_uint(r1) & 0xffff0000u;
     const float r2 = r1 - __uint_as_float(b1);
-    const int lane = ((k >> 3) & 1) * 32 + (n & 31);
-    uint16_t* dst = Wx + (((((int64_t)(n >> 7) * ksteps + (k >> 4)) * 4 + ((n >> 5) & 3)) * 3) * 64 + lane) * 8 + (k & 7);
+    const int lane = k32 ? ((k >> 3) & 3) * 16 + (n & 15) : ((k >> 3) & 1) * 32 + (n & 31);
+    const int64_t frag = k32 ? (((int64_t)(n >> 7) * (ksteps >> 1) + (k >> 5)) * 8 + ((n >> 4) & 7)) * 3
+                             : (((int64_t)(n >> 7) * ksteps + (k >> 4)) * 4 + ((n >> 5) & 3)) * 3;
+    uint16_t* dst = Wx + (frag * 64 + lane) * 8 + (k & 7);
     dst[0] = (uint16_t)(b0 >> 16);
     dst[512] = (uint16_t)(b1 >> 16);
     dst[1024] = (uint16_t)(__float_as_uint(r2) >> 16);
@@ -230,7 +232,9 @@
 }
 PackItem pack_first_w(const float* w, float* wf, int Cout, int Cin) { return item(PACK_FIRST_W, w, wf, Cout, Cin); }
 PackItem pack_first_mfma(const float* w, float* wfm, int Cout, int Cin) { return item(PACK_FIRST_MFMA, w, wfm, Cout, Cin); }
-PackItem pack_convt_x3(const float* w, float* Wx, int Cin, int Cout, int dgrad) { return item(PACK_CONVT_X3, w, Wx, Cout, Cin, 0, 0, dgrad); }
+PackItem pack_convt_x3(const float* w, float* Wx, int Cin, int Cout, int dgrad, int k32) {
+  return item(PACK_CONVT_X3, w, Wx, Cout, Cin, 0, 0, dgrad, k32);
+}
 PackItem pack_bias_tile(const float* bias, float* shift, int C, int reps) { return item(PACK_BIAS_TILE, bias, shift, C, reps); }
 PackItem pack_dgrad_panel(const float* w, float* wp, int Cout, int Cin, int Cop, int KS, int Kp) {
   return item(PACK_DGRAD_PANEL, w, wp, Cout, Cin, Cop, Kp, KS);
@@ -251,7 +255,7 @@
     case PACK_WINO: pack_wino_w_body(t.w, t.U, t.Cout, t.Cin, t.Cp, t.Np, t.dgrad, t.mode, vblock, vgrid); break;
     case PACK_FIRST_W: pack_first_w_body(t.w, t.U, t.Cout, t.Cin, vblock, vgrid); break;
     case PACK_FIRST_MFMA: pack_first_mfma_body(t.w, reinterpret_cast<uint16_t*>(t.U), t.Cout, t.Cin, vblock, vgrid); break;
-    case PACK_CONVT_X3: pack_convt_x3_body(t.w, reinterpret_cast<uint16_t*>(t.U), t.Cin, t.Cout, t.dgrad, vblock, vgrid); break;
+    case PACK_CONVT_X3: pack_convt_x3_body(t.w, reinterpret_cast<uint16_t*>(t.U), t.Cin, t.Cout, t.dgrad, t.mode, vblock, vgrid); break;
     case PACK_BIAS_TILE: pack_bias_tile_body(t.w, t.U, t.Cout, t.Cin, vblock, vgrid); break;
     case PACK_DGRAD_PANEL: pack_dgrad_w_body(t.w, t.U, t.Cout, t.Cin, t.Cp, t.dgrad, t.Np, vblock, vgrid); break;
     case PACK_CONV_PANEL:
@@ -278,7 +282,7 @@
     case PACK_FIRST_W: work = 9 * 4 * (int64_t)t.Cout; break;
     case PACK_FIRST_MFMA: work = 2 * 64 * 8; break;
     case PACK_CONVT_X3:
-      if ((t.Cin & (t.dgrad ? 63 : 15)) || (t.Cout & 31)) return 0;
+      if ((t.Cin & (t.dgrad ? 63 : t.mode ? 31 : 15)) || (t.Cout & 31) || (t.mode && t.dgrad)) return 0;
       work = (int64_t)t.Cin * t.Cout * 4;
       break;
     case PACK_BIAS_TILE: work = (int64_t)t.Cout * t.Cin; break;
```

Result: no change. 812.5 (median of 6 runs) (+0.8%).
